# prismformore/Multi-Task-Transformer

Measured on AMD Instinct MI355X. Metric: training images/sec (512x512, 6 tasks), higher is better.
Workload: dtype f32(bf16x3)

## Files before the change

include/mtt_hip.h:

```cpp
#ifndef MTT_HIP_H
#define MTT_HIP_H

#include <stddef.h>
#include <stdint.h>

#ifdef __cplusplus
extern "C" {
#endif

#define MTT_ABI_VERSION 17

enum { MTT_F32 = 0, MTT_BF16 = 1, MTT_SPLIT = 2 };
enum { MTT_PREC_BF16 = 0, MTT_PREC_X3 = 1 };
enum { MTT_E_BADARG = -1, MTT_E_ALIGN = -2, MTT_E_UNSUPPORTED = -3 };

enum {
  MTT_OP_K = 0,
  MTT_OP_R = 1,
  MTT_OP_CONV_K = 2,
  MTT_OP_CONV_R = 3
};
enum { MTT_ACT_NONE = 0, MTT_ACT_GELU = 1, MTT_ACT_RELU = 2, MTT_ACT_GELU_BWD = 3, MTT_ACT_RELU_BWD = 4,
       MTT_ACT_GELU_DAUX = 5 ,
       MTT_ACT_MUL_AUX = 6    };
enum { MTT_STORE_ROWS = 0, MTT_STORE_PIXSHUF2 = 1 };
enum { MTT_GEMM_AUTO = 0,
       MTT_GEMM_GENERAL = 1           ,
       MTT_GEMM_DMA256 = 3            ,
       MTT_GEMM_DMA128 = 4            ,
       MTT_GEMM_GENERAL_EPILOGUE = 11  };
enum { MTT_ATTN_AUTO = 0, MTT_ATTN_PLAIN = 1,
       MTT_ATTN_FAST_V0 = 2 ,
       MTT_ATTN_FAST_V1 = 3  };

typedef struct {
  int32_t H, W;
  int32_t C;
  int32_t Cp;
  int32_t dil;
  int32_t flip;
} mtt_conv_geom;

typedef struct {
  const void* A; const void* B; void* D;
  int32_t M, N, K;
  int32_t a_op, b_op;
  int32_t a_dtype, b_dtype, d_dtype;
  int32_t prec;
  int64_t lda, ldb, ldd;
  int32_t a_mb; int64_t a_bs;
  int32_t d_mb; int64_t d_bs;
  int32_t batch, batch_inner;
  int64_t a_zo, a_zi, b_zo, b_zi, d_zo, d_zi;
  mtt_conv_geom conv;
  float alpha;
  const float* colscale; const float* colshift; int64_t col_zo, col_zi;
  int32_t act;
  const void* aux_in; void* aux_out; int32_t aux_dtype; int64_t ldaux; int64_t aux_zo, aux_zi;
  const float* rowscale; int32_t n_prompt;
  const float* resid; int64_t ldr; int32_t r_mb; int64_t r_bs; int64_t r_zo, r_zi;
  int32_t n_store;
  int32_t store_mode;
  int32_t ps_H, ps_W, ps_Co;
  int32_t variant;
  const void* A_lo; const void* B_lo; void* D_lo;
  float* colsum_out; float* colsum_ws;
  const float* a_scale; const float* a_shift; int32_t a_act; void* a_aux16; int64_t ld_a16;
} mtt_gemm_desc;
size_t mtt_gemm_colsum_ws_floats(const mtt_gemm_desc* d);

int mtt_abi_version(void);
size_t mtt_desc_size(int which);
int mtt_gemm(const mtt_gemm_desc* d, void* stream);
int mtt_gemm_variant(const mtt_gemm_desc* d);

typedef struct {
  const void* qkv; void* out; float* rawlog; float* lse;
  int32_t B, N, nH, T;
  int32_t dtype, prec;
  float scale;
  int32_t variant;
  const void* qkv_lo; void* out_lo;
} mtt_attn_desc;
int mtt_attn_fwd(const mtt_attn_desc* d, void* stream);
int mtt_attn_bwd(const mtt_attn_desc* d, const void* dout, const float* drawlog, void* dqkv, float* stat, void* stream);

typedef struct {
  const void* S; void* P; const void* dP; void* dS; const float* extra;
  int64_t rows, cols, ld; int32_t s_dtype, p_dtype; float scale;
  int64_t rows_per_mat; int32_t extra_rows; int64_t extra_ld;
} mtt_softmax_desc;
int mtt_softmax_fwd(const mtt_softmax_desc* d, void* stream);
int mtt_softmax_bwd(const mtt_softmax_desc* d, void* stream);

typedef struct {
  const float* x; void* y; const float* gamma; const float* beta; float* mean; float* rstd;
  const void* dy; float* dx; float* dgamma; float* dbeta;
  int64_t rows; int32_t C; int64_t ldx, ldy; int32_t y_dtype; float eps;
  const float* dx_in;
  float* ws;
  void* y_lo;
  float* y32; int64_t ldy32;
} mtt_ln_desc;
size_t mtt_layernorm_bwd_ws_floats(int64_t rows, int32_t C);
int mtt_layernorm_fwd(const mtt_ln_desc* d, void* stream);
int mtt_layernorm_bwd(const mtt_ln_desc* d, void* stream);

int mtt_patchify16(const float* img, void* cols, int B, int H, int W, int out_dtype, void* stream);

typedef struct {
  const void* q; const void* xn; float* rawchan;
  int32_t B, T, N, C, h, w, nh, nw; int32_t dtype; int64_t ldq;
  float* ws;
  const void* xn_lo;
} mtt_chanlogit_desc;
size_t mtt_chan_logits_ws_floats(const mtt_chanlogit_desc* d);
int mtt_chan_logits(const mtt_chanlogit_desc* d, void* stream);
int mtt_chan_logits_bwd(const mtt_chanlogit_desc* d, const float* drawchan, void* dq, int dq_dtype, float* dxn, void* stream);

typedef struct {
  const float* x; int64_t x_ld, x_bs; const float* rawlog; const float* rawchan; void* out;
  int32_t B, T, N, C, h, w, nh, nw; int32_t out_dtype;
  int32_t hg;
  void* out_lo;
} mtt_modulate_desc;
int mtt_modulate(const mtt_modulate_desc* d, void* stream);
size_t mtt_modulate_bwd_ws_floats(const mtt_modulate_desc* d);
int mtt_modulate_bwd(const mtt_modulate_desc* d, const void* dout, float* dx, float* drawlog, float* drawchan, float* ws, void* stream);

typedef struct {
  const void* fea; void* out; const float* wmix;
  int32_t T, B; int64_t rows_per_b, ld; int32_t C; int32_t fea_dtype; int32_t accumulate;
  int32_t out_dtype;
} mtt_ctr_desc;
int mtt_ctr_mix(const mtt_ctr_desc* d, void* stream);
size_t mtt_ctr_dw_ws_floats(const mtt_ctr_desc* d);
int mtt_ctr_dw(const mtt_ctr_desc* d, const float* dout, float* dwmix, float* ws, void* stream);

typedef struct {
  const float* rawlog; const float* w0; const float* b0; const float* w2; const float* b2; float* wmix;
  int32_t B, T, nH; int64_t N;
} mtt_ctrw_desc;
int mtt_ctr_weights(const mtt_ctrw_desc* d, void* stream);
int mtt_ctr_weights_bwd(const mtt_ctrw_desc* d, const float* dwmix, float* drawlog, float* dw0, float* db0, float* dw2, float* db2, void* stream);

typedef struct {
  const float* pred; const void* target; const float* weight; float* out; float* sum; float* ws;
  int64_t N; int32_t C; int32_t kind; int32_t wmode; float gamma, alpha, beta;
} mtt_detloss_desc;
size_t mtt_detloss_ws_floats(const mtt_detloss_desc* d);
int mtt_detloss_fwd(const mtt_detloss_desc* d, void* stream);
int mtt_detloss_bwd(const mtt_detloss_desc* d, const float* gscale, const float* gelem, float scale, float* dpred, void* stream);

typedef struct {
  const void* in; void* out; int32_t B, C, Hin, Win, Hout, Wout; int64_t ld_in, ld_out;
  int32_t in_dtype, out_dtype; int32_t out_nchw; int32_t accumulate;
} mtt_resize_desc;
int mtt_bilinear_fwd(const mtt_resize_desc* d, void* stream);
int mtt_bilinear_bwd(const mtt_resize_desc* d, void* stream);

typedef struct {
  const void* x; void* y; const void* dy; void* dx;
  float* mean_out; float* m2_out; const float* mean; const float* rstd; const float* gamma; const float* beta;
  float* dsum; float* dsumxh;
  int64_t rows; int32_t C; int64_t ld; int32_t dtype; int32_t act;
// ... 249 lines not shown
```

multi-task-transformer_amd/_lib.py:

```python
import ctypes as C
import os

import torch

_HERE = os.path.dirname(os.path.abspath(__file__))
LIB_PATH = os.path.join(_HERE, "libmtt_hip.so")

ABI_VERSION = 17
F32, BF16, SPLIT = 0, 1, 2
PREC_BF16, PREC_X3 = 0, 1
OP_K, OP_R, OP_CONV_K, OP_CONV_R = 0, 1, 2, 3
ACT_NONE, ACT_GELU, ACT_RELU, ACT_GELU_BWD, ACT_RELU_BWD, ACT_GELU_DAUX, ACT_MUL_AUX = 0, 1, 2, 3, 4, 5, 6
STORE_ROWS, STORE_PIXSHUF2 = 0, 1
GEMM_AUTO, GEMM_GENERAL, GEMM_DMA256, GEMM_DMA128, GEMM_GENERAL_EPILOGUE = 0, 1, 3, 4, 11
ATTN_AUTO, ATTN_PLAIN = 0, 1

i32, i64, f32, ptr = C.c_int32, C.c_int64, C.c_float, C.c_void_p


class ConvGeom(C.Structure):
    _fields_ = [("H", i32), ("W", i32), ("C", i32), ("Cp", i32), ("dil", i32), ("flip", i32)]


class GemmDesc(C.Structure):
    _fields_ = [
        ("A", ptr), ("B", ptr), ("D", ptr),
        ("M", i32), ("N", i32), ("K", i32),
        ("a_op", i32), ("b_op", i32),
        ("a_dtype", i32), ("b_dtype", i32), ("d_dtype", i32),
        ("prec", i32),
        ("lda", i64), ("ldb", i64), ("ldd", i64),
        ("a_mb", i32), ("a_bs", i64),
        ("d_mb", i32), ("d_bs", i64),
        ("batch", i32), ("batch_inner", i32),
        ("a_zo", i64), ("a_zi", i64), ("b_zo", i64), ("b_zi", i64), ("d_zo", i64), ("d_zi", i64),
        ("conv", ConvGeom),
        ("alpha", f32),
        ("colscale", ptr), ("colshift", ptr), ("col_zo", i64), ("col_zi", i64),
        ("act", i32),
        ("aux_in", ptr), ("aux_out", ptr), ("aux_dtype", i32), ("ldaux", i64), ("aux_zo", i64), ("aux_zi", i64),
        ("rowscale", ptr), ("n_prompt", i32),
        ("resid", ptr), ("ldr", i64), ("r_mb", i32), ("r_bs", i64), ("r_zo", i64), ("r_zi", i64),
        ("n_store", i32), ("store_mode", i32),
        ("ps_H", i32), ("ps_W", i32), ("ps_Co", i32),
        ("variant", i32),
        ("A_lo", ptr), ("B_lo", ptr), ("D_lo", ptr),
        ("colsum_out", ptr), ("colsum_ws", ptr),
        ("a_scale", ptr), ("a_shift", ptr), ("a_act", i32), ("a_aux16", ptr), ("ld_a16", i64),
    ]


class AttnDesc(C.Structure):
    _fields_ = [("qkv", ptr), ("out", ptr), ("rawlog", ptr), ("lse", ptr),
                ("B", i32), ("N", i32), ("nH", i32), ("T", i32), ("dtype", i32), ("prec", i32), ("scale", f32),
                ("variant", i32), ("qkv_lo", ptr), ("out_lo", ptr)]


class SoftmaxDesc(C.Structure):
    _fields_ = [("S", ptr), ("P", ptr), ("dP", ptr), ("dS", ptr), ("extra", ptr),
                ("rows", i64), ("cols", i64), ("ld", i64), ("s_dtype", i32), ("p_dtype", i32), ("scale", f32),
                ("rows_per_mat", i64), ("extra_rows", i32), ("extra_ld", i64)]


class LnDesc(C.Structure):
    _fields_ = [("x", ptr), ("y", ptr), ("gamma", ptr), ("beta", ptr), ("mean", ptr), ("rstd", ptr),
                ("dy", ptr), ("dx", ptr), ("dgamma", ptr), ("dbeta", ptr),
                ("rows", i64), ("C", i32), ("ldx", i64), ("ldy", i64), ("y_dtype", i32), ("eps", f32), ("dx_in", ptr), ("ws", ptr),
                ("y_lo", ptr), ("y32", ptr), ("ldy32", i64)]


class ChanLogitDesc(C.Structure):
    _fields_ = [("q", ptr), ("xn", ptr), ("rawchan", ptr),
                ("B", i32), ("T", i32), ("N", i32), ("C", i32), ("h", i32), ("w", i32), ("nh", i32), ("nw", i32),
                ("dtype", i32), ("ldq", i64), ("ws", ptr), ("xn_lo", ptr)]


class ModulateDesc(C.Structure):
    _fields_ = [("x", ptr), ("x_ld", i64), ("x_bs", i64), ("rawlog", ptr), ("rawchan", ptr), ("out", ptr),
                ("B", i32), ("T", i32), ("N", i32), ("C", i32), ("h", i32), ("w", i32), ("nh", i32), ("nw", i32),
                ("out_dtype", i32), ("hg", i32), ("out_lo", ptr)]


class CtrDesc(C.Structure):
    _fields_ = [("fea", ptr), ("out", ptr), ("wmix", ptr), ("T", i32), ("B", i32), ("rows_per_b", i64), ("ld", i64),
                ("C", i32), ("fea_dtype", i32), ("accumulate", i32), ("out_dtype", i32)]


class ResizeDesc(C.Structure):
    _fields_ = [("in_", ptr), ("out", ptr), ("B", i32), ("C", i32), ("Hin", i32), ("Win", i32), ("Hout", i32), ("Wout", i32),
                ("ld_in", i64), ("ld_out", i64), ("in_dtype", i32), ("out_dtype", i32), ("out_nchw", i32), ("accumulate", i32)]


class BnDesc(C.Structure):
    _fields_ = [("x", ptr), ("y", ptr), ("dy", ptr), ("dx", ptr),
                ("mean_out", ptr), ("m2_out", ptr), ("mean", ptr), ("rstd", ptr), ("gamma", ptr), ("beta", ptr),
                ("dsum", ptr), ("dsumxh", ptr),
                ("rows", i64), ("C", i32), ("ld", i64), ("dtype", i32), ("act", i32),
                ("Z", i32), ("x_zs", i64), ("p_zs", i64), ("g_dtype", i32)]


class DwconvDesc(C.Structure):
    _fields_ = [("x", ptr), ("w", ptr), ("y", ptr), ("scale", ptr), ("shift", ptr),
                ("Z", i32), ("B", i32), ("H", i32), ("W", i32), ("ld", i64), ("dtype", i32)]


class PoolDesc(C.Structure):
    _fields_ = [("x", ptr), ("y", ptr), ("B", i32), ("H", i32), ("W", i32), ("k", i32), ("ld", i64), ("dtype", i32)]


class LnMtDesc(C.Structure):
    _fields_ = [("x", ptr), ("y", ptr), ("gamma", ptr), ("beta", ptr), ("rows", i64), ("T", i32), ("D", i32),
                ("ldx", i64), ("ldy", i64), ("y_dtype", i32), ("eps", f32)]


class AttnMsgDesc(C.Structure):
    _fields_ = [("cur", ptr), ("prev", ptr), ("out", ptr), ("w", ptr), ("bias", ptr),
                ("B", i32), ("heads", i32), ("T", i32), ("qh", i32), ("qw", i32), ("K", i32), ("ldk", i64), ("ldkp", i64)]


class ConvtDesc(C.Structure):
    _fields_ = [("yall", ptr), ("out", ptr), ("bias", ptr), ("B", i32), ("H", i32), ("W", i32), ("Cop", i32),
                ("dtype", i32), ("out_dtype", i32)]


class UpconvDesc(C.Structure):
    _fields_ = [("z", ptr), ("y", ptr), ("bias", ptr), ("colscale", ptr),
                ("Z", i32), ("B", i32), ("h", i32), ("w", i32), ("C", i32), ("Cp", i32),
                ("z_dtype", i32), ("y_dtype", i32), ("act", i32)]


class AdamDesc(C.Structure):
    _fields_ = [("grads", ptr), ("params", ptr), ("exp_avg", ptr), ("exp_avg_sq", ptr), ("numel", ptr),
                ("chunk_tensor", ptr), ("chunk_off", ptr), ("n_chunks", i32),
                ("max_norm", f32), ("step_size", f32), ("beta1", f32), ("beta2", f32), ("eps", f32), ("weight_decay", f32),
                ("inv_sqrt_bc2", f32), ("hyper", ptr), ("ws", ptr)]


class LossDesc(C.Structure):
# ... 327 lines not shown
```

multi-task-transformer_amd/autograd_path.py:

```python
import math

import torch
import torch.distributed as dist
import torch.nn as nn
from torch.autograd import Function

from . import bn as bn_mod
from . import _lib, ops
from ._lib import ACT_GELU, ACT_GELU_BWD, ACT_GELU_DAUX, ACT_MUL_AUX, ACT_NONE, F32, OP_CONV_R, OP_K, OP_R, dtype_code

pitch = ops.pitch
SPLITK_MIN_ROWS = 4096
WGRAD_MAX_SLICES, WGRAD_TARGET_WGS = 192, 512


def _gemm(A, B, D, M, N, K, prec, **kw):
    args = dict(A=A, B=B, D=D, M=M, N=N, K=K, a_op=OP_K, b_op=OP_K, a_dtype=dtype_code(A), b_dtype=dtype_code(B),
                d_dtype=dtype_code(D), prec=prec.code, batch=1, batch_inner=1, alpha=1.0)
    args.update(kw)
    ops.call("gemm", **args)
    return D


def _colsum(x2d, cols):
# ... 59 lines not shown
def _wgrad_batched(dy, x, N, Kp, M, prec, Z, lda, ldb, a_zo, b_zo, a0=0, b0=0):
    A = dy.reshape(-1)[a0:] if a0 else dy
    B = x.reshape(-1)[b0:] if b0 else x
    p256 = (-(-N // 256)) * (-(-Kp // 256))
    if (prec.name == "bf16" and FAST_BWD and dy.dtype == torch.bfloat16 and x.dtype == torch.bfloat16 and M >= SPLITK_MIN_ROWS
            and min(N, Kp) >= FAST_MIN_DIM and 100 * N * Kp >= 45 * p256 * 65536 and lda % 8 == 0 and ldb % 8 == 0):
        S = _tn_splits(Z * p256, M)
        c = (M // S) // 64 * 64
        if c >= 512:
            nz = M // c
            rem = M - nz * c
            slabs = torch.empty(Z, nz + (1 if rem else 0), N, Kp, dtype=torch.float32, device=dy.device)
            SS = slabs.shape[1]
            _gemm(A, B, slabs, N, Kp, c, prec, a_op=OP_R, b_op=OP_R, lda=lda, ldb=ldb, ldd=Kp, batch=Z * nz, batch_inner=nz,
                  a_zo=a_zo, a_zi=c * lda, b_zo=b_zo, b_zi=c * ldb, d_zo=SS * N * Kp, d_zi=N * Kp)
            if rem:
                _gemm(dy.reshape(-1)[a0 + nz * c * lda:], x.reshape(-1)[b0 + nz * c * ldb:], slabs[:, nz], N, Kp, rem, prec, a_op=OP_R,
                      b_op=OP_R, lda=lda, ldb=ldb, ldd=Kp, batch=Z, a_zo=a_zo, b_zo=b_zo, d_zo=SS * N * Kp)
            return slabs.sum(1)
    tiles = Z * (-(-N // 128)) * (-(-Kp // 128))
    S = _n_splits(tiles, M // SPLIT_ROW_UNIT)
    if S == 1:
        dW = torch.empty(Z, N, Kp, dtype=torch.float32, device=dy.device)
        _gemm(A, B, dW, N, Kp, M, prec, a_op=OP_R, b_op=OP_R, lda=lda, ldb=ldb, ldd=Kp, batch=Z, a_zo=a_zo, b_zo=b_zo, d_zo=N * Kp)
        return dW
    c = (M // S) // 8 * 8
    rem = M - c * S
    slabs = torch.empty(Z, S + (1 if rem else 0), N, Kp, dtype=torch.float32, device=dy.device)
    SS = slabs.shape[1]
    _gemm(A, B, slabs, N, Kp, c, prec, a_op=OP_R, b_op=OP_R, lda=lda, ldb=ldb, ldd=Kp, batch=Z * S, batch_inner=S,
          a_zo=a_zo, a_zi=c * lda, b_zo=b_zo, b_zi=c * ldb, d_zo=SS * N * Kp, d_zi=N * Kp)
    if rem:
        _gemm(dy.reshape(-1)[a0 + c * S * lda:], x.reshape(-1)[b0 + c * S * ldb:], slabs[:, S], N, Kp, rem, prec, a_op=OP_R, b_op=OP_R,
              lda=lda, ldb=ldb, ldd=Kp, batch=Z, a_zo=a_zo, b_zo=b_zo, d_zo=SS * N * Kp)
    return slabs.sum(1)


def _pad_last(t, width):
    out = torch.zeros(t.shape[:-1] + (width,), dtype=t.dtype, device=t.device)
    out[..., :t.shape[-1]] = t
    return out


N_CUS = 256


def _tn_splits(tiles, rows, max_splits=32):
    best, cost = 2, None
    for S in range(2, max_splits + 1):
        t = -(-tiles * S // N_CUS) / S * rows * 131072 / 4.7e12 + S * tiles * 65536 * 8 / 4e12
        if cost is None or t < cost:
            best, cost = S, t
    return best


def _wgrad_tn(dy, x, N, Kp, prec):
    rows = dy.shape[0]
    lda, ldb = dy.stride(0), x.stride(0)
    tiles = -(-N // 256) * -(-Kp // 256)
    if tiles < 192 and rows >= 4096:
        S = _tn_splits(tiles, rows)
        c = (rows // S) // 64 * 64
        if c >= 512:
            nz = rows // c
            rem = rows - nz * c
            slabs = torch.empty(nz + (1 if rem else 0), N, Kp, dtype=torch.float32, device=dy.device)
            _gemm(dy, x, slabs, N, Kp, c, prec, a_op=OP_R, b_op=OP_R, lda=lda, ldb=ldb, ldd=Kp, batch=nz, a_zo=c * lda, b_zo=c * ldb, d_zo=N * Kp)
            if rem:
                _gemm(dy[nz * c:], x[nz * c:], slabs[nz], N, Kp, rem, prec, a_op=OP_R, b_op=OP_R, lda=lda, ldb=ldb, ldd=Kp)
            return slabs.sum(0)
    dW = torch.empty(N, Kp, dtype=torch.float32, device=dy.device)
    return _gemm(dy, x, dW, N, Kp, rows, prec, a_op=OP_R, b_op=OP_R, lda=lda, ldb=ldb, ldd=Kp)


def _enc_wgrad(dy, x, N, Kp, prec, bias=True):
    db = _colsum(dy, N) if bias else None
    if (prec.name == "bf16" and FAST_BWD and N >= FAST_MIN_DIM and Kp >= FAST_MIN_DIM and dy.shape[0] >= FAST_MIN_ROWS
            and N % 8 == 0 and dy.stride(0) % 8 == 0):
        if dy.dtype == torch.bfloat16 and x.dtype == torch.bfloat16:
            return _wgrad_tn(dy, x, N, Kp, prec), db
    return _wgrad(dy, x, N, Kp, prec), db


def _enc_dgrad(dy, weight, wpack2d, M, N_in, K_out, prec, out_dtype, tag, colsum=False, **epi):
    if colsum:
        if prec.name == "bf16" and (dy.dtype != torch.bfloat16 or wpack2d.dtype != torch.bfloat16):
            dx = _enc_dgrad(dy, weight, wpack2d, M, N_in, K_out, prec, out_dtype, tag, **epi)
            return dx, _colsum(dx, N_in)
        cs = torch.empty(N_in, dtype=torch.float32, device=dy.device)
        epi = dict(epi, colsum_out=cs, colsum_ws=ops.ws_for("gemm_colsum", dy.device, M=M, N=N_in))
        return _enc_dgrad(dy, weight, wpack2d, M, N_in, K_out, prec, out_dtype, tag, **epi), cs
    if prec.name == "bf16" and FAST_BWD and dy.dtype == torch.bfloat16 and K_out % 64 == 0 and N_in >= FAST_MIN_DIM:
        wT = ops.pack_linear_T(weight, torch.bfloat16, tag)
        dx = torch.empty(M, N_in, dtype=out_dtype, device=dy.device)
        return _gemm(dy, wT, dx, M, N_in, K_out, prec, lda=dy.stride(0), ldb=wT.stride(0), ldd=N_in, n_store=N_in, **epi)
    return _dgrad(dy, wpack2d, M, N_in, K_out, prec, out_dtype, **epi)


FAST_BWD = True
GELU_DAUX = True
FAST_MIN_DIM, FAST_MIN_ROWS = 256, 1024


def _dgrad(dy, wpack2d, M, N_in, K_out, prec, out_dtype, **epi):
    dx = torch.empty(M, N_in, dtype=out_dtype, device=dy.device)
    return _gemm(dy, wpack2d, dx, M, N_in, K_out, prec, b_op=OP_R, lda=dy.stride(0), ldb=wpack2d.stride(0), ldd=N_in,
                 n_store=N_in, **epi)


def layernorm(x, gamma, beta, eps, prec, out_dtype, keep):
    if keep:
        return LayerNormFn.apply(x, gamma, beta, eps, prec, out_dtype)
    return ops.layernorm(x, gamma, beta, eps, prec, out_dtype=out_dtype)[0]


class LayerNormFn(Function):
    @staticmethod
    def forward(ctx, x, gamma, beta, eps, prec, out_dtype):
        y, mean, rstd = ops.layernorm(x, gamma, beta, eps, prec, save_stats=True, out_dtype=out_dtype)
        ctx.save_for_backward(x, gamma, mean, rstd)
        ctx.eps = eps
        return y

    @staticmethod
    def backward(ctx, dy):
        x, gamma, mean, rstd = ctx.saved_tensors
        dy = dy.contiguous()
        dx, dg, db = torch.zeros_like(x), torch.empty_like(gamma), torch.empty_like(gamma)
        ops.call("layernorm_bwd", x=x, dy=dy, gamma=gamma, mean=mean, rstd=rstd, dx=dx, dgamma=dg, dbeta=db,
                 rows=x.shape[0], C=x.shape[1], ldx=x.stride(0), ldy=dy.stride(0), y_dtype=dtype_code(dy), eps=ctx.eps,
                 ws=ops.ln_bwd_ws(x.shape[0], x.shape[1], x.device))
        return dx, dg, db, None, None, None


def attention_bwd(qkv, dao, drawlog, B, N, nH, T, prec):
    C, Np, Z = nH * 64, pitch(N), B * nH
    dev, adt = qkv.device, prec.adt
    scale = 64 ** -0.5
    S = torch.empty(Z, N, Np, dtype=adt, device=dev)
    zS = dict(batch=Z, batch_inner=nH, d_zo=nH * N * Np, d_zi=N * Np)
    zq = dict(a_zo=N * 3 * C, a_zi=64)
    _gemm(qkv, qkv[:, C:], S, N, N, 64, prec, lda=3 * C, ldb=3 * C, ldd=Np, b_zo=N * 3 * C, b_zi=64, n_store=Np, **zq, **zS)
    ops.call("softmax_fwd", S=S, P=S, rows=Z * N, cols=N, ld=Np, s_dtype=dtype_code(S), p_dtype=dtype_code(S), scale=scale)
    dP = torch.empty(Z, N, Np, dtype=adt, device=dev)
    _gemm(dao, qkv[:, 2 * C:], dP, N, N, 64, prec, lda=C, ldb=3 * C, ldd=Np, a_zo=N * C, a_zi=64, b_zo=N * 3 * C, b_zi=64,
          n_store=Np, **zS)
    ops.call("softmax_bwd", P=S, dP=dP, dS=dP, extra=drawlog, rows=Z * N, cols=N, ld=Np, s_dtype=dtype_code(S),
             p_dtype=dtype_code(S), scale=scale, rows_per_mat=N, extra_rows=T if drawlog is not None else 0, extra_ld=N)
    dqkv = torch.empty(B * N, 3 * C, dtype=adt, device=dev)
    zP = dict(batch=Z, batch_inner=nH, a_zo=nH * N * Np, a_zi=N * Np, d_zo=N * 3 * C, d_zi=64)
    _gemm(S, dao, dqkv[:, 2 * C:], N, 64, N, prec, a_op=OP_R, b_op=OP_R, lda=Np, ldb=C, ldd=3 * C, b_zo=N * C, b_zi=64, **zP)
    _gemm(dP, qkv[:, C:], dqkv, N, 64, N, prec, b_op=OP_R, lda=Np, ldb=3 * C, ldd=3 * C, b_zo=N * 3 * C, b_zi=64, **zP)
    _gemm(dP, qkv, dqkv[:, C:], N, 64, N, prec, a_op=OP_R, b_op=OP_R, lda=Np, ldb=3 * C, ldd=3 * C, b_zo=N * 3 * C, b_zi=64, **zP)
    return dqkv


HEAD_DGRAD_DMA = True
FLASH_BWD = True


def attention_bwd_flash(qkv, ao, lse, dao, drawlog, B, N, nH, T, prec):
    dqkv = torch.empty_like(qkv)
    dsum = torch.empty(B, nH, 2, (N + 3) // 4 * 4, dtype=torch.float32, device=qkv.device)
    ops.call("attn_bwd", qkv=qkv, out=ao, rawlog=None, lse=lse, B=B, N=N, nH=nH, T=T, dtype=dtype_code(qkv), prec=prec.code,
             scale=64 ** -0.5, xargs=[dao, drawlog, dqkv, dsum])
    return dqkv


def _ln_bwd_join(dres, x, dy, gamma, mean, rstd, eps):
    dg, db = torch.empty_like(gamma), torch.empty_like(gamma)
    out = torch.empty_like(dres)
    ops.call("layernorm_bwd", x=x, dy=dy, gamma=gamma, mean=mean, rstd=rstd, dx=out, dx_in=dres, dgamma=dg, dbeta=db,
             rows=x.shape[0], C=x.shape[1], ldx=x.stride(0), ldy=dy.stride(0), y_dtype=dtype_code(dy), eps=eps,
             ws=ops.ln_bwd_ws(x.shape[0], x.shape[1], x.device))
    return out, dg, db


def attn_half(XT, g1, b1, eps, Wqkv, bqkv, Wproj, bproj, Wtt, btt, Wtt1, btt1, rowscale, geo, prec, tag, *, keep, gp=None):
    B, N, nH, T, h, w, nwin = geo[:7]
    side = geo[7] if len(geo) > 7 else True
    pe, pa, ps = gp or (prec, prec, prec)
    assert not keep or pe.name == pa.name == ps.name == prec.name, "per-group precisions are inference-only"
    C, hw = nH * 64, h * w
    chan = Wtt is not None
    split = prec.split
    odt = "split" if split else prec.adt
    xn, mean, rstd = ops.layernorm(XT, g1, b1, eps, prec, save_stats=keep, out_dtype=odt)
    wq = ops.pack_linear([Wqkv], pe, tag + ('qkv',), split=split)
    wp = ops.pack_linear([Wproj], pe, tag + ('proj',), split=split)
    qkv = ops.linear(xn, wq, 3 * C, pe, bias=bqkv[None], out_dtype=odt)[0]
    flash = keep and (split or (FLASH_BWD and prec.name == "bf16" and qkv.dtype == torch.bfloat16))
    if not split and pa.adt != qkv.dtype:
        q16 = ops.cast2d(qkv, qkv.shape[0], 3 * C, 3 * C, pa.adt, ldd=3 * C)
        ao16, rawlog, lse = ops.attention(q16, B, N, nH, T, pa)
        ao = ops.cast2d(ao16, ao16.shape[0], C, C, prec.adt, ldd=C)
    else:
        ao, rawlog, lse = ops.attention(qkv, B, N, nH, T, pa, want_lse=flash)
    XT2 = torch.empty_like(XT)
    rows = dict(d_rows=(N, N * C, C), M=B * N) if keep or rowscale is not None else {}
    ops.linear(ao, wp, C, pe, bias=bproj[None], out=XT2, resid=XT, rowscale=rowscale, n_prompt=T, **rows)
    cq = wt = wt1 = xp32 = rawchan = None
    if chan:
        wt = ops.pack_linear([Wtt], ps, tag + ('tt',))
        wt1 = ops.pack_linear([Wtt1], ps, tag + ('tt1',))
        if split:
            xp32 = ops.prompt_rows32(xn, B, N, T, C)
            cq = ops.linear(xp32, wt, hw, ps, bias=btt[None], M=B * T)[0]
        else:
            cq = ops.linear(xn, wt, hw, ps, bias=btt[None], a_rows=(T, N * C, C), M=B * T)[0]
        if side:
            xnc = xn if split or ps.adt == xn.dtype else ops.cast2d(xn, xn.shape[0], C, C, ps.adt, ldd=C)
            rawchan = ops.chan_logits(cq, xnc, B, T, N, C, (h, w), (nwin, nwin))
        pr = XT2.view(B, N, C)[:, :T]
        ops.linear(cq, wt1, C, ps, bias=btt1[None], out=pr, d_rows=(T, N * C, C), resid=pr, rowscale=rowscale, n_prompt=T, M=B * T)
    saved = (XT, g1, mean, rstd, ops._hi(xn), ops._hi(qkv), ops._hi(ao), ops._hi(wq), ops._hi(wp), rowscale, lse, cq, wt, wt1, xp32) if keep else None
    return (XT2, rawlog, rawchan), saved


def mlp_half(XT2, g2, b2n, eps, W1, b1, W2, b2, rowscale, geo, prec, tag, *, keep, pe=None):
    B, N, T = geo
    pe = pe or prec
    assert not keep or pe.name == prec.name
    C, Hd = W1.shape[1], W1.shape[0]
    split = prec.split and ((C % 64 == 0 and Hd % 64 == 0) if MLP_SPLIT_RULE64 else (ops.split_gemm_ok(C) and ops.split_gemm_ok(Hd)))
    odt = "split" if split else prec.adt
    xn2, mean, rstd = ops.layernorm(XT2, g2, b2n, eps, prec, save_stats=keep, out_dtype=odt)
    w1 = ops.pack_linear([W1], pe, tag + ('fc1',), split=split)
    w2 = ops.pack_linear([W2], pe, tag + ('fc2',), split=split)
    z = torch.empty(B * N, Hd, dtype=prec.bwd.adt, device=XT2.device) if keep else None
    daux = keep and GELU_DAUX and z.dtype == torch.bfloat16
    hmid = ops.linear(xn2, w1, Hd, pe, bias=b1[None], act=ACT_GELU_DAUX if daux else ACT_GELU, aux_out=z, out_dtype=odt)[0]
    XT3 = torch.empty_like(XT2)
    rows = dict(d_rows=(N, N * C, C), M=B * N) if keep or rowscale is not None else {}
    ops.linear(hmid, w2, C, pe, bias=b2[None], out=XT3, resid=XT2, rowscale=rowscale, n_prompt=T, **rows)
    saved = (XT2, g2, mean, rstd, ops._hi(xn2), z, ops._hi(hmid), ops._hi(w1), ops._hi(w2), rowscale) if keep else None
    return XT3, saved


class AttnHalfFn(Function):

    @staticmethod
    def forward(ctx, XT, g1, b1, eps, Wqkv, bqkv, Wproj, bproj, Wtt, btt, Wtt1, btt1, rowscale, geo, prec, tag):
        (XT2, rawlog, rawchan), saved = attn_half(XT, g1, b1, eps, Wqkv, bqkv, Wproj, bproj, Wtt, btt, Wtt1, btt1, rowscale, geo, prec, tag, keep=True)
        ctx.save_for_backward(*saved)
        ctx.geo, ctx.prec, ctx.eps, ctx.chan = geo, prec, eps, Wtt is not None
        ctx.params = (Wqkv, Wproj, Wtt, Wtt1)
        ctx.set_materialize_grads(False)
        z = torch.zeros(0, device=XT.device)
        return XT2, (rawlog if rawlog is not None else z), (rawchan if rawchan is not None else z)

    @staticmethod
    def backward(ctx, dXT2, drawlog, drawchan):
        XT, g1, mean, rstd, xn, qkv, ao, wq, wp, rowscale, lse, cq, wt, wt1, xp32 = ctx.saved_tensors
        Wqkv_, Wproj_, Wtt_, Wtt1_ = ctx.params
        B, N, nH, T, h, w, nwin = ctx.geo[:7]
        prec, C, M, hw = ctx.prec.bwd, nH * 64, B * N, h * w
        xn_c = xn
        if dXT2 is None:
            dXT2 = torch.zeros_like(XT)
        dXT2 = dXT2.contiguous()
        g, dbproj = _scaled_colsum(dXT2, rowscale, N, T, prec)
        dWproj, _ = _enc_wgrad(g, ao, C, C, prec, bias=False)
        dao = _enc_dgrad(g, Wproj_, wp[0], M, C, C, prec, prec.adt, 'proj')
        dl = drawlog.contiguous() if (T > 0 and drawlog is not None and drawlog.numel()) else None
        if lse is not None:
            dqkv = attention_bwd_flash(qkv, ao, lse, dao, dl, B, N, nH, T, prec)
        else:
            dqkv = attention_bwd(qkv, dao, dl, B, N, nH, T, prec)
        dWqkv, dbqkv = _enc_wgrad(dqkv, xn, 3 * C, C, prec)
        dxn = _enc_dgrad(dqkv, Wqkv_, wq[0], M, C, 3 * C, prec, torch.float32, 'qkv')
        dWtt = dbtt = dWtt1 = dbtt1 = None
        if ctx.chan:
            hwp = cq.shape[-1]
            gp = dXT2.view(B, N, C)[:, :T].reshape(B * T, C)
            if rowscale is not None:
                gp = gp * rowscale[:, 0].repeat_interleave(T)[:, None]
            dWtt1 = _wgrad(gp, cq, C, hwp, prec)[:, :hw]
            dbtt1 = _colsum(gp, C)
            fast_tt = prec.name == "bf16" and FAST_BWD and hwp == hw and hw >= FAST_MIN_DIM and C >= FAST_MIN_DIM and C % 64 == 0
            if fast_tt:
                gp16 = ops.cast_rows(gp, torch.bfloat16)
                dcq = _enc_dgrad(gp16, Wtt1_, wt1[0], B * T, hwp, C, prec, torch.float32, 'tt1')
            else:
                dcq = _dgrad(gp, wt1[0], B * T, hwp, C, prec, torch.float32)
            if drawchan is not None and drawchan.numel():
                dq2 = torch.zeros(B * T, hwp, dtype=torch.float32, device=xn.device)
                cqb = cq if cq.dtype == xn_c.dtype else ops.cast_rows(cq, xn_c.dtype)
                ops.call("chan_logits_bwd", q=cqb, xn=xn_c, rawchan=None, B=B, T=T, N=N, C=C, h=h, w=w, nh=nwin, nw=nwin,
                         dtype=dtype_code(xn_c), ldq=hwp, xargs=[drawchan.contiguous(), dq2, F32, dxn])
                dcq = dcq + dq2
            xnp = xp32 if xp32 is not None else xn_c.view(B, N, C)[:, :T].reshape(B * T, C)
            dWtt = _wgrad(dcq, xnp, hw, C, prec)[:, :C]
            dbtt = _colsum(dcq, hw)
            dp = dxn.view(B, N, C)[:, :T]
            if fast_tt:
                dcq16 = ops.cast_rows(dcq, torch.bfloat16)
                wT = ops.pack_linear_T(Wtt_, torch.bfloat16, 'tt')
                _gemm(dcq16, wT, dp, B * T, C, hw, prec, lda=hwp, ldb=hw, ldd=C, d_mb=T, d_bs=N * C,
                      resid=dp, r_mb=T, r_bs=N * C, ldr=C, n_store=C)
            else:
                _gemm(dcq, wt[0], dp, B * T, C, hw, prec, b_op=OP_R, lda=hwp, ldb=wt.shape[-1], ldd=C, d_mb=T, d_bs=N * C,
                      resid=dp, r_mb=T, r_bs=N * C, ldr=C, n_store=C)
        dXT, dg1, db1 = _ln_bwd_join(dXT2, XT, dxn, g1, mean, rstd, ctx.eps)
        return (dXT, dg1, db1, None, dWqkv, dbqkv, dWproj, dbproj, dWtt, dbtt, dWtt1, dbtt1, None, None, None, None)


class MlpHalfFn(Function):

    @staticmethod
    def forward(ctx, XT2, g2, b2n, eps, W1, b1, W2, b2, rowscale, geo, prec, tag):
        XT3, saved = mlp_half(XT2, g2, b2n, eps, W1, b1, W2, b2, rowscale, geo, prec, tag, keep=True)
        ctx.save_for_backward(*saved)
        ctx.geo, ctx.prec, ctx.eps, ctx.daux = geo, prec, eps, GELU_DAUX and saved[5].dtype == torch.bfloat16
        ctx.params = (W1, W2)
        return XT3

    @staticmethod
    def backward(ctx, dXT3):
        XT2, g2, mean, rstd, xn2, z, hmid, w1, w2, rowscale = ctx.saved_tensors
        B, N, T = ctx.geo
        prec, M = ctx.prec.bwd, B * N
        C, Hd = xn2.shape[1], z.shape[1]
        dXT3 = dXT3.contiguous()
        g, db2 = _scaled_colsum(dXT3, rowscale, N, T, prec)
        W1_, W2_ = ctx.params
        dW2, _ = _enc_wgrad(g, hmid, C, Hd, prec, bias=False)
        dz, db1 = _enc_dgrad(g, W2_, w2[0], M, Hd, C, prec, prec.adt, 'fc2', colsum=True, act=ACT_MUL_AUX if ctx.daux else ACT_GELU_BWD, aux_in=z,
                             aux_dtype=dtype_code(z), ldaux=Hd)
        dW1, _ = _enc_wgrad(dz, xn2, Hd, C, prec, bias=False)
        dxn2 = _enc_dgrad(dz, W1_, w1[0], M, C, Hd, prec, prec.adt, 'fc1')
        dXT2, dg2, dbn2 = _ln_bwd_join(dXT3, XT2, dxn2, g2, mean, rstd, ctx.eps)
        return dXT2, dg2, dbn2, None, dW1, db1, dW2, db2, None, None, None, None


def block_attn(keep, gp, *args):
    return AttnHalfFn.apply(*args) if keep else attn_half(*args, keep=False, gp=gp)[0]


def block_mlp(keep, pe, *args):
    return MlpHalfFn.apply(*args) if keep else mlp_half(*args, keep=False, pe=pe)[0]


def patch_embed(img, Wpe, bpe, pos, first, geo, prec, tag, pe=None):
    B, N, T, hw = geo
    C = Wpe.shape[0]
    XT = torch.empty(B * N, C, dtype=torch.float32, device=img.device)
    XT.view(B, N, C)[:, :T] = first
    cols = ops.patchify(img.float(), prec)
    wpe = ops.pack_linear([Wpe], pe or prec, tag)
    ops.linear(cols, wpe, C, pe or prec, bias=bpe[None], out=XT.view(B, N, C)[:, T:], d_rows=(hw, N * C, C),
               resid=pos[0, 1:], r_rows=(hw, 0, C), M=B * hw)
    return XT, cols


class PatchEmbedFn(Function):

    @staticmethod
    def forward(ctx, img, Wpe, bpe, pos, prompts, geo, prec):
        XT, cols = patch_embed(img, Wpe, bpe, pos, prompts, geo, prec, 'pe')
        ctx.save_for_backward(cols)
        ctx.geo, ctx.prec, ctx.wshape = geo, prec, Wpe.shape
        return XT

    @staticmethod
    def backward(ctx, dXT):
        (cols,) = ctx.saved_tensors
        B, N, T, hw = ctx.geo
        C = ctx.wshape[0]
        d3 = dXT.contiguous().view(B, N, C)
        dpatch = d3[:, T:].reshape(B * hw, C)
        dW = _wgrad(dpatch, cols, C, 768, ctx.prec.bwd).view(ctx.wshape)
        db = _colsum(dpatch, C)
        dpos = torch.zeros(1, hw + 1, C, dtype=torch.float32, device=dXT.device)
        dpos[0, 1:] = d3[:, T:].sum(0)
        return None, dW, db, dpos, d3[:, :T].sum(0), None, None


class ModulateFn(Function):

    @staticmethod
    def forward(ctx, xsrc, rawlog, rawchan, geo, prec, split=False):
        B, N, T, C, h, w, nwin = geo[:7]
        hg = geo[7] if len(geo) > 7 else 0
        mod = ops.modulate(xsrc.view(B, N, C)[:, T:], C, N * C, rawlog, rawchan, B, T, N, C, (h, w), (nwin, nwin), prec, hg=hg, split=split)
        ctx.save_for_backward(xsrc, rawlog, rawchan)
        ctx.geo = geo
        if split:
            ctx.mark_non_differentiable(mod.lo)
            ctx.set_materialize_grads(False)
            return mod.hi, mod.lo
        return mod

    @staticmethod
    def backward(ctx, dmod, *_):
        xsrc, rawlog, rawchan = ctx.saved_tensors
        B, N, T, C, h, w, nwin = ctx.geo[:7]
        hg = ctx.geo[7] if len(ctx.geo) > 7 else 0
        dmod = dmod.contiguous()
        dx = torch.empty_like(xsrc)
        dx.view(B, N, C)[:, :T].zero_()
        dl, dc = torch.zeros_like(rawlog), torch.empty_like(rawchan)
        ops.call("modulate_bwd", x=xsrc.view(B, N, C)[:, T:], x_ld=C, x_bs=N * C, rawlog=rawlog, rawchan=rawchan, out=None,
                 B=B, T=T, N=N, C=C, h=h, w=w, nh=nwin, nw=nwin, out_dtype=dtype_code(dmod), hg=hg,
                 xargs=[dmod, dx.view(B, N, C)[:, T:], dl, dc, ops.ws_for("modulate_bwd", dmod.device, B=B, T=T, C=C, h=h, w=w, nh=nwin, nw=nwin)])
        return dx, dl, dc, None, None, None


MLP_SPLIT_RULE64 = False
AUTO_SPLIT = True
AUTO_SPLIT_MIN_ROWS = 2048


class BLinearFn(Function):
# ... 640 lines not shown
```

multi-task-transformer_amd/csrc/attn_bwd.hip:

```cpp
#include "mtt_device.h"
#include <type_traits>

#ifndef MTT_ABWD_TILES
#define MTT_ABWD_TILES 1
#endif
#ifndef MTT_ABWD_STATDMA
#define MTT_ABWD_STATDMA 1
#endif
#ifndef MTT_ABWD_DQSTAT
#define MTT_ABWD_DQSTAT 1
#endif

namespace {

constexpr int HD = 64;
constexpr int KTILE = 64 * HD * 2;
constexpr float LOG2E = 1.4426950408889634f;

struct BwdP {
  const bf16_t* qkv; const bf16_t* dout; const float* stat; const float* drawlog; bf16_t* dqkv;
  int B, N, nH, T, Np; float scale;
  const bf16_t* out; const float* lse; float* stat_w;
};

MTT_DEV float dot8_bf16(const u32x4& a, const u32x4& g) {
  float s = 0.f;
#pragma unroll
  for (int j = 0; j < 4; ++j) s += lo_of(a[j]) * lo_of(g[j]) + hi_of(a[j]) * hi_of(g[j]);
  return s;
}

__global__ __launch_bounds__(256) void attn_stat_kernel(const bf16_t* out, const bf16_t* dout, const float* lse, float* stat, int B, int N,
                                                        int nH, int Np) {
  const int C8 = nH * 8;
  const int64_t total = (int64_t)B * N * C8;
  const int64_t t = (int64_t)blockIdx.x * 256 + threadIdx.x;
  float s = 0.f;
  if (t < total) {
    const u32x4 a = *(const u32x4*)(out + t * 8), g = *(const u32x4*)(dout + t * 8);
    s = dot8_bf16(a, g);
  }
  s += __shfl_xor(s, 1, 64); s += __shfl_xor(s, 2, 64); s += __shfl_xor(s, 4, 64);
  if (t < total && (threadIdx.x & 7) == 0) {
    const int64_t tok = t / C8;
    const int h = (int)(t % C8) >> 3;
    const int b = (int)(tok / N), n = (int)(tok % N);
    float* row = stat + ((int64_t)b * nH + h) * 2 * Np;
    row[n] = s;
    row[Np + n] = lse[((int64_t)b * nH + h) * N + n] * LOG2E;
    if (n == N - 1)
      for (int k = N; k < Np; ++k) { row[k] = 0.f; row[Np + k] = 0.f; }
  }
}

MTT_DEV u32x4 perm_frag(const unsigned char* tile, int row, int ks, int lg) {
  const u32x2 lo = *(const u32x2*)(tile + lds_off(row, 4 * ks + (lg >> 1)) + (lg & 1) * 8);
  const u32x2 hi = *(const u32x2*)(tile + lds_off(row, 4 * ks + 2 + (lg >> 1)) + (lg & 1) * 8);
  return (u32x4){lo[0], lo[1], hi[0], hi[1]};
}

template <bool TR>
MTT_DEV void store_units(unsigned char* rowmajor, unsigned char* transposed, const u32x4 (&sh)[4], int kq, int rb) {
#pragma unroll
  for (int i = 0; i < 4; ++i) *(u32x4*)(rowmajor + lds_off(kq * 4 + i, rb)) = sh[i];
  if (TR) {
    u32x2 piece[8];
    transpose4x8(sh, piece);
#pragma unroll
    for (int j = 0; j < 8; ++j) *(u32x2*)(transposed + lds_off(rb * 8 + j, kq >> 1) + (kq & 1) * 8) = piece[j];
  }
}

__device__ __attribute__((aligned(32))) const unsigned g_bwd_zero_page[8] = {0u, 0u, 0u, 0u, 0u, 0u, 0u, 0u};
MTT_DEV int bwd_swz(int row) { return (((row >> 1) & 3) << 1) | ((row >> 3) & 1); }
MTT_DEV void bwd_glds16(const bf16_t* src, unsigned char* lds_wave_base) {
  __builtin_amdgcn_global_load_lds((const __attribute__((address_space(1))) void*)src,
                                   (__attribute__((address_space(3))) void*)lds_wave_base, 16, 0, 0);
}
MTT_DEV void bwd_glds4(const float* src, unsigned char* lds_wave_base) {
  __builtin_amdgcn_global_load_lds((const __attribute__((address_space(1))) void*)src,
                                   (__attribute__((address_space(3))) void*)lds_wave_base, 4, 0, 0);
}
using BwdDyn = std::integral_constant<int, -1>;
using BwdNo = std::integral_constant<int, 0>;
using BwdYes = std::integral_constant<int, 1>;
template <int OFF>
MTT_DEV u32x2 bwd_ds_read_tr16(unsigned addr) {
  u32x2 r;
  asm volatile("ds_read_b64_tr_b16 %0, %1 offset:%2" : "=v"(r) : "v"(addr), "n"(OFF) : "memory");
  return r;
}
template <int OFF>
MTT_DEV f32x4 bwd_ds_read_f4(unsigned addr) {
  f32x4 r;
  asm volatile("ds_read_b128 %0, %1 offset:%2" : "=v"(r) : "v"(addr), "n"(OFF) : "memory");
  return r;
}
#define BWD_TRW(x) "+v"(x)
#define BWD_WAIT_TR8(a, b)                                                                                                              \
  asm volatile("s_waitcnt lgkmcnt(0)" : BWD_TRW(a[0]), BWD_TRW(a[1]), BWD_TRW(a[2]), BWD_TRW(a[3]), BWD_TRW(b[0]), BWD_TRW(b[1]), BWD_TRW(b[2]), BWD_TRW(b[3]) :: "memory")
#define BWD_WAIT_TR16(a, b, c, d)                                                                                                       \
  asm volatile("s_waitcnt lgkmcnt(0)" : BWD_TRW(a[0]), BWD_TRW(a[1]), BWD_TRW(a[2]), BWD_TRW(a[3]), BWD_TRW(b[0]), BWD_TRW(b[1]), BWD_TRW(b[2]), BWD_TRW(b[3]), \
               BWD_TRW(c[0]), BWD_TRW(c[1]), BWD_TRW(c[2]), BWD_TRW(c[3]), BWD_TRW(d[0]), BWD_TRW(d[1]), BWD_TRW(d[2]), BWD_TRW(d[3]) :: "memory")
#define BWD_WAIT_TR16_F4(a, b, c, d, e, f)                                                                                              \
  asm volatile("s_waitcnt lgkmcnt(0)" : BWD_TRW(a[0]), BWD_TRW(a[1]), BWD_TRW(a[2]), BWD_TRW(a[3]), BWD_TRW(b[0]), BWD_TRW(b[1]), BWD_TRW(b[2]), BWD_TRW(b[3]), \
               BWD_TRW(c[0]), BWD_TRW(c[1]), BWD_TRW(c[2]), BWD_TRW(c[3]), BWD_TRW(d[0]), BWD_TRW(d[1]), BWD_TRW(d[2]), BWD_TRW(d[3]),                       \
               BWD_TRW(e[0]), BWD_TRW(e[1]), BWD_TRW(f[0]), BWD_TRW(f[1]) :: "memory")

template <int VER>
__global__ __launch_bounds__(256, 2) void attn_bwd_dq_kernel(const BwdP p) {
  extern __shared__ __attribute__((aligned(16))) unsigned char smem[];
  constexpr int STAGE = (VER == 2 ? 2 : 3) * KTILE;
  const int nqb = (p.N + 127) / 128;
  const int wi = xcd_remap(blockIdx.x, gridDim.x);
  const int qb = wi % nqb, bh_ = wi / nqb;
  const int h = bh_ % p.nH, b = bh_ / p.nH;
  const int N = p.N, C = p.nH * HD;
  const int tid = threadIdx.x, lane = tid & 63, wave = tid >> 6;
  const int li = lane & 15, lg = lane >> 4;
  const int64_t tok0 = (int64_t)b * N;
  const int64_t bh = (int64_t)b * p.nH + h;
  const int q0 = qb * 128 + wave * 32;
  const bool active = q0 < N;

  u32x4 qf[2][2], gf[2][2], dummy;
  float lse2[2], Dq[2];
#pragma unroll
  for (int sub = 0; sub < 2; ++sub) {
    const int qrow = q0 + sub * 16 + li;
    const bool ok = qrow < N;
#pragma unroll
    for (int kh = 0; kh < 2; ++kh) {
      Raw8<false> r;
      load8_raw<false>(p.qkv, (tok0 + qrow) * 3 * C + h * HD + kh * 32 + lg * 8, ok, r);
      cvt8<false, false>(ok, r, qf[sub][kh], dummy);
      load8_raw<false>(p.dout, (tok0 + qrow) * C + h * HD + kh * 32 + lg * 8, ok, r);
      cvt8<false, false>(ok, r, gf[sub][kh], dummy);
    }
    if constexpr (VER == 2 && MTT_ABWD_DQSTAT) {
      float c[2];
#pragma unroll
      for (int kh = 0; kh < 2; ++kh) {
        Raw8<false> r;
        u32x4 of;
        load8_raw<false>(p.out, (tok0 + qrow) * C + h * HD + kh * 32 + lg * 8, ok, r);
        cvt8<false, false>(ok, r, of, dummy);
        c[kh] = dot8_bf16(of, gf[sub][kh]);
        c[kh] += __shfl_xor(c[kh], 16, 64);
        c[kh] += __shfl_xor(c[kh], 32, 64);
      }
      Dq[sub] = c[0] + c[1];
      lse2[sub] = ok ? p.lse[bh * N + qrow] * LOG2E : 0.f;
      if (ok && lg == 0) {
        p.stat_w[bh * 2 * p.Np + qrow] = Dq[sub];
        p.stat_w[bh * 2 * p.Np + p.Np + qrow] = lse2[sub];
      }
    } else {
      Dq[sub] = ok ? p.stat[bh * 2 * p.Np + qrow] : 0.f;
      lse2[sub] = ok ? p.stat[bh * 2 * p.Np + p.Np + qrow] : 0.f;
    }
  }
  if constexpr (VER == 2 && MTT_ABWD_DQSTAT) {
    if (qb == nqb - 1 && tid < p.Np - N) {
      p.stat_w[bh * 2 * p.Np + N + tid] = 0.f;
      p.stat_w[bh * 2 * p.Np + p.Np + N + tid] = 0.f;
    }
  }

  const bool isK = tid < 128;
  const int kq = tid & 15, rb = (tid >> 4) & 7;
  Raw8<false> raw[4];
  unsigned okm = 0;
  auto stage_load = [&](int kv0) {
    if (VER >= 1 && kv0 + 64 <= N) {
      okm = 0xfu;
#pragma unroll
      for (int i = 0; i < 4; ++i)
        raw[i].r0 = *(const u32x4*)(p.qkv + ((tok0 + kv0 + kq * 4 + i) * 3 * C + (isK ? C : 2 * C) + h * HD + rb * 8));
      return;
    }
    okm = 0;
#pragma unroll
    for (int i = 0; i < 4; ++i) {
      const int key = kv0 + kq * 4 + i;
      const bool ok = key < N;
      okm |= (ok ? 1u : 0u) << i;
      load8_raw<false>(p.qkv, (tok0 + key) * 3 * C + (isK ? C : 2 * C) + h * HD + rb * 8, ok, raw[i]);
    }
  };
  auto stage_store = [&](unsigned char* st) {
    u32x4 sh[4];
    if (VER >= 1 && okm == 0xfu) {
#pragma unroll
      for (int i = 0; i < 4; ++i) sh[i] = raw[i].r0;
    } else {
#pragma unroll
      for (int i = 0; i < 4; ++i) cvt8<false, false>((okm >> i) & 1u, raw[i], sh[i], dummy);
    }
    if (isK) store_units<true>(st, st + KTILE, sh, kq, rb);
    else store_units<false>(st + 2 * KTILE, nullptr, sh, kq, rb);
  };

  int dma_off[4], dma_row[2];
  uint64_t zpage = 0;
// ... 259 lines not shown
    for (int i = 0; i < 4; ++i) {
      const int row = q0 + kq * 4 + i;
      const bool ok = row < N;
      okm |= (ok ? 1u : 0u) << i;
      if (isQ) load8_raw<false>(p.qkv, (tok0 + row) * 3 * C + h * HD + rb * 8, ok, raw[i]);
      else load8_raw<false>(p.dout, (tok0 + row) * C + h * HD + rb * 8, ok, raw[i]);
    }
  };
  auto stage_store = [&](unsigned char* st) {
    u32x4 sh[4];
    if (VER >= 1 && okm == 0xfu) {
#pragma unroll
      for (int i = 0; i < 4; ++i) sh[i] = raw[i].r0;
    } else {
#pragma unroll
      for (int i = 0; i < 4; ++i) cvt8<false, false>((okm >> i) & 1u, raw[i], sh[i], dummy);
    }
    unsigned char* base = isQ ? st : st + 2 * KTILE;
    store_units<true>(base, base + KTILE, sh, kq, rb);
  };

  int dma_off[4], dma_row[2];
  uint64_t zpage = 0;
  unsigned taddr[4];
  const unsigned char* faddr[2];
  if (VER == 2) {
    zpage = (uint64_t)(uintptr_t)g_bwd_zero_page;
    asm volatile("" : "+s"(zpage));
#pragma unroll
    for (int i = 0; i < 2; ++i) {
      const int r = wave * 16 + i * 8 + (lane >> 3), pc = lane & 7;
      dma_row[i] = r;
      dma_off[i] = r * 3 * C + ((pc ^ bwd_swz(r)) & 7) * 8;
      dma_off[2 + i] = r * C + ((pc ^ bwd_swz(r)) & 7) * 8;
    }
    const int trow = 4 * lg + (li >> 2);
#pragma unroll
    for (int dt = 0; dt < 4; ++dt)
      taddr[dt] = (unsigned)(uintptr_t)smem + (unsigned)(trow * 128 + (((2 * dt + ((li & 3) >> 1)) ^ bwd_swz(trow)) & 7) * 16 + (li & 1) * 8);
#pragma unroll
    for (int kh = 0; kh < 2; ++kh) faddr[kh] = smem + li * 128 + (((kh * 4 + lg) ^ bwd_swz(li)) & 7) * 16;
  }
  const float* Drow = p.stat + bh * 2 * p.Np;
  const float* Lrow = Drow + p.Np;
  constexpr int STAT_LDS = 2 * STAGE, STAT_STAGE = 2 * 64 * 4;
  const unsigned saddr = (unsigned)(uintptr_t)smem + (unsigned)(lg * 16);
  auto dma_issue = [&](unsigned char* st, unsigned char* sst, int q0) {
    if (MTT_ABWD_STATDMA && __builtin_amdgcn_readfirstlane(wave) < 2) {
      const float* src = (wave ? Lrow : Drow) + q0 + lane;
      if (q0 + 64 > p.Np) src = q0 + lane < p.Np ? src : (const float*)(uintptr_t)zpage;
      bwd_glds4(src, sst + wave * 256);
    }
    const bf16_t* baseQ = p.qkv + ((tok0 + q0) * 3 * C + h * HD);
    const bf16_t* baseG = p.dout + ((tok0 + q0) * C + h * HD);
    unsigned char* dQ = st + wave * 2048;
    unsigned char* dG = st + KTILE + wave * 2048;
    if (q0 + 64 <= N) {
#pragma unroll
      for (int i = 0; i < 2; ++i) bwd_glds16(baseQ + dma_off[i], dQ + i * 1024);
#pragma unroll
      for (int i = 0; i < 2; ++i) bwd_glds16(baseG + dma_off[2 + i], dG + i * 1024);
    } else {
#pragma unroll
      for (int i = 0; i < 2; ++i) {
        const bool ok = q0 + dma_row[i] < N;
        bwd_glds16((const bf16_t*)(uintptr_t)(ok ? (uint64_t)(uintptr_t)(baseQ + dma_off[i]) : zpage), dQ + i * 1024);
      }
#pragma unroll
      for (int i = 0; i < 2; ++i) {
        const bool ok = q0 + dma_row[i] < N;
        bwd_glds16((const bf16_t*)(uintptr_t)(ok ? (uint64_t)(uintptr_t)(baseG + dma_off[2 + i]) : zpage), dG + i * 1024);
      }
    }
  };

  f32x4 dk[2][4], dv[2][4];
#pragma unroll
  for (int kt = 0; kt < 2; ++kt)
#pragma unroll
    for (int t = 0; t < 4; ++t) { dk[kt][t] = (f32x4){0.f, 0.f, 0.f, 0.f}; dv[kt][t] = (f32x4){0.f, 0.f, 0.f, 0.f}; }
  const float sc2 = p.scale * LOG2E, inv_scale = 1.0f / p.scale;

  const int nq = (N + 63) / 64;
  if (VER == 2) {
    dma_issue(smem, smem + STAT_LDS, 0);
    asm volatile("s_waitcnt vmcnt(0)" ::: "memory");
  } else {
    stage_load(0);
    stage_store(smem);
  }
  __syncthreads();

  auto tile = [&](auto stage_tag, auto ragged_tag, auto first_tag, int j) {
    constexpr int ST = decltype(stage_tag)::value;
    constexpr int RG = decltype(ragged_tag)::value, FT = decltype(first_tag)::value;
    const bool more = RG != 1 && j + 1 < nq;
    if (more) {
      if (VER == 2) dma_issue(smem + (1 - ST) * STAGE, smem + STAT_LDS + (1 - ST) * STAT_STAGE, (j + 1) * 64);
      else stage_load((j + 1) * 64);
    }
    const unsigned char* Qh = smem + (ST < 0 ? (j & 1) : ST) * STAGE;
    const unsigned char* Qt = Qh + KTILE;
    const unsigned char* Gh = Qh + 2 * KTILE;
    const unsigned char* Gt = Qh + 3 * KTILE;
    const int q0 = j * 64;
    if (active) {
      const bool full = RG < 0 ? q0 + 64 <= N : RG == 0;
      const bool add_raw = FT != 0 && p.drawlog != nullptr && (FT > 0 || j == 0) && p.T > 0;
#pragma unroll
      for (int ks = 0; ks < 2; ++ks) {
        if (RG != 0 && q0 + 32 * ks >= N) continue;
        f32x4 s[2][2], dp[2][2];
        f32x4 D4[2], L4[2];
        u32x2 qtl[4], qth[4], gtl[4], gth[4];
        if constexpr (VER == 2) {
          constexpr bool LATE = RG == 1;
          u32x4 qa[2][2], ga[2][2];
          auto read_stat = [&]() {
#pragma unroll
            for (int q2 = 0; q2 < 2; ++q2) {
              D4[q2] = bwd_ds_read_f4<STAT_LDS + ST * STAT_STAGE>(saddr + (ks ? 128 : 0) + q2 * 64);
              L4[q2] = bwd_ds_read_f4<STAT_LDS + ST * STAT_STAGE + 256>(saddr + (ks ? 128 : 0) + q2 * 64);
            }
          };
          auto read_tr = [&]() {
            if (ks == 0) {
#pragma unroll
              for (int dt = 0; dt < 4; ++dt) {
                qtl[dt] = bwd_ds_read_tr16<ST * STAGE>(taddr[dt]); qth[dt] = bwd_ds_read_tr16<ST * STAGE + 16 * 128>(taddr[dt]);
                gtl[dt] = bwd_ds_read_tr16<ST * STAGE + KTILE>(taddr[dt]); gth[dt] = bwd_ds_read_tr16<ST * STAGE + KTILE + 16 * 128>(taddr[dt]);
              }
            } else {
#pragma unroll
              for (int dt = 0; dt < 4; ++dt) {
                qtl[dt] = bwd_ds_read_tr16<ST * STAGE + 32 * 128>(taddr[dt]); qth[dt] = bwd_ds_read_tr16<ST * STAGE + 48 * 128>(taddr[dt]);
                gtl[dt] = bwd_ds_read_tr16<ST * STAGE + KTILE + 32 * 128>(taddr[dt]); gth[dt] = bwd_ds_read_tr16<ST * STAGE + KTILE + 48 * 128>(taddr[dt]);
              }
            }
          };
          auto wait_reads = [&]() {
            if constexpr (MTT_ABWD_STATDMA) BWD_WAIT_TR16_F4(qtl, qth, gtl, gth, D4, L4);
            else BWD_WAIT_TR16(qtl, qth, gtl, gth);
          };
          if constexpr (MTT_ABWD_STATDMA && !LATE) read_stat();
#pragma unroll
          for (int q2 = 0; q2 < 2; ++q2) {
            if constexpr (!MTT_ABWD_STATDMA) {
              const int qr = q0 + (2 * ks + q2) * 16 + lg * 4;
              D4[q2] = qr < p.Np ? *(const f32x4*)(Drow + qr) : (f32x4){0.f, 0.f, 0.f, 0.f};
              L4[q2] = qr < p.Np ? *(const f32x4*)(Lrow + qr) : (f32x4){0.f, 0.f, 0.f, 0.f};
            }
#pragma unroll
            for (int kh = 0; kh < 2; ++kh) {
              qa[q2][kh] = *(const u32x4*)(faddr[kh] + ST * STAGE + q2 * 2048 + (ks ? 4096 : 0));
              ga[q2][kh] = *(const u32x4*)(faddr[kh] + ST * STAGE + KTILE + q2 * 2048 + (ks ? 4096 : 0));
            }
          }
          if constexpr (!LATE) { read_tr(); wait_reads(); }
          __builtin_amdgcn_s_setprio(1);
#pragma unroll
          for (int q2 = 0; q2 < 2; ++q2) {
#pragma unroll
            for (int kt = 0; kt < 2; ++kt) { s[q2][kt] = (f32x4){0.f, 0.f, 0.f, 0.f}; dp[q2][kt] = (f32x4){0.f, 0.f, 0.f, 0.f}; }
#pragma unroll
            for (int kh = 0; kh < 2; ++kh)
#pragma unroll
              for (int kt = 0; kt < 2; ++kt) {
                s[q2][kt] = mfma16(qa[q2][kh], kf[kt][kh], s[q2][kt]);
                dp[q2][kt] = mfma16(ga[q2][kh], vf[kt][kh], dp[q2][kt]);
              }
          }
          __builtin_amdgcn_s_setprio(0);
          if constexpr (LATE) {
            if constexpr (MTT_ABWD_STATDMA) read_stat();
            read_tr();
            wait_reads();
          }
        } else {
        if (VER >= 1) __builtin_amdgcn_s_setprio(1);
#pragma unroll
        for (int q2 = 0; q2 < 2; ++q2) {
          const int qs = 2 * ks + q2;
          const int qr = q0 + qs * 16 + lg * 4;
          D4[q2] = qr < p.Np ? *(const f32x4*)(Drow + qr) : (f32x4){0.f, 0.f, 0.f, 0.f};
          L4[q2] = qr < p.Np ? *(const f32x4*)(Lrow + qr) : (f32x4){0.f, 0.f, 0.f, 0.f};
#pragma unroll
          for (int kt = 0; kt < 2; ++kt) { s[q2][kt] = (f32x4){0.f, 0.f, 0.f, 0.f}; dp[q2][kt] = (f32x4){0.f, 0.f, 0.f, 0.f}; }
#pragma unroll
          for (int kh = 0; kh < 2; ++kh) {
            const u32x4 qa = *(const u32x4*)(Qh + lds_off(qs * 16 + li, kh * 4 + lg));
            const u32x4 ga = *(const u32x4*)(Gh + lds_off(qs * 16 + li, kh * 4 + lg));
#pragma unroll
            for (int kt = 0; kt < 2; ++kt) {
              s[q2][kt] = mfma16(qa, kf[kt][kh], s[q2][kt]);
              dp[q2][kt] = mfma16(ga, vf[kt][kh], dp[q2][kt]);
            }
          }
        }
        if (VER >= 1) __builtin_amdgcn_s_setprio(0);
        }
        u32x4 pb[2], dsb[2];
#pragma unroll
        for (int kt = 0; kt < 2; ++kt) {
          float pv[2][4], ds[2][4];
#pragma unroll
          for (int q2 = 0; q2 < 2; ++q2) {
            const float lr[4] = {L4[q2][0], L4[q2][1], L4[q2][2], L4[q2][3]};
            const float dr[4] = {D4[q2][0], D4[q2][1], D4[q2][2], D4[q2][3]};
#pragma unroll
            for (int r = 0; r < 4; ++r) {
              pv[q2][r] = __builtin_amdgcn_exp2f(fmaf(s[q2][kt][r], sc2, -lr[r]));
              if (!full && q0 + (2 * ks + q2) * 16 + lg * 4 + r >= N) pv[q2][r] = 0.f;
              ds[q2][r] = pv[q2][r] * (dp[q2][kt][r] - dr[r]);
            }
          }
          if (add_raw && ks == 0) {
            const int key = key0 + kt * 16 + li;
#pragma unroll
            for (int r = 0; r < 4; ++r) {
              const int q = lg * 4 + r;
              if (q < p.T && key < N) ds[0][r] += p.drawlog[(bh * p.T + q) * N + key] * inv_scale;
            }
          }
          pb[kt] = (u32x4){pack2(pv[0][0], pv[0][1]), pack2(pv[0][2], pv[0][3]), pack2(pv[1][0], pv[1][1]), pack2(pv[1][2], pv[1][3])};
          dsb[kt] = (u32x4){pack2(ds[0][0], ds[0][1]), pack2(ds[0][2], ds[0][3]), pack2(ds[1][0], ds[1][1]), pack2(ds[1][2], ds[1][3])};
        }
        if (VER >= 1) __builtin_amdgcn_s_setprio(1);
#pragma unroll
        for (int dt = 0; dt < 4; ++dt) {
          u32x4 ga, qa;
          if constexpr (VER == 2) {
            ga = (u32x4){gtl[dt][0], gtl[dt][1], gth[dt][0], gth[dt][1]};
            qa = (u32x4){qtl[dt][0], qtl[dt][1], qth[dt][0], qth[dt][1]};
          } else {
            ga = perm_frag(Gt, dt * 16 + li, ks, lg);
            qa = perm_frag(Qt, dt * 16 + li, ks, lg);
          }
#pragma unroll
          for (int kt = 0; kt < 2; ++kt) {
            dv[kt][dt] = mfma16(ga, pb[kt], dv[kt][dt]);
            dk[kt][dt] = mfma16(qa, dsb[kt], dk[kt][dt]);
          }
        }
        if (VER >= 1) __builtin_amdgcn_s_setprio(0);
      }
    }
    if (more) {
      if (VER == 2) asm volatile("s_waitcnt vmcnt(0)" ::: "memory");
      else stage_store(smem + (ST < 0 ? ((j + 1) & 1) : (1 - ST)) * STAGE);
    }
    __syncthreads();
  };
  if (VER == 2 && MTT_ABWD_TILES) {
    const int nfull = N / 64;
    if (nfull >= 1) tile(BwdNo{}, BwdNo{}, BwdYes{}, 0);
    else tile(BwdNo{}, BwdYes{}, BwdYes{}, 0);
    for (int j = 1; j < nfull; j += 2) {
      tile(BwdYes{}, BwdNo{}, BwdNo{}, j);
      if (j + 1 < nfull) tile(BwdNo{}, BwdNo{}, BwdNo{}, j + 1);
    }
    if (nfull >= 1 && nfull < nq) {
      if (nfull & 1) tile(BwdYes{}, BwdYes{}, BwdNo{}, nfull);
      else tile(BwdNo{}, BwdYes{}, BwdNo{}, nfull);
    }
  } else if (VER >= 1) {
    for (int j = 0; j < nq; j += 2) {
      tile(BwdNo{}, BwdDyn{}, BwdDyn{}, j);
      if (j + 1 < nq) tile(BwdYes{}, BwdDyn{}, BwdDyn{}, j + 1);
    }
  } else {
    for (int j = 0; j < nq; ++j) tile(BwdDyn{}, BwdDyn{}, BwdDyn{}, j);
  }
  int tid_e = tid;
  asm volatile("" : "+v"(tid_e));
  const int li_e = tid_e & 15, lg_e = (tid_e >> 4) & 3, key0_e = kb * 128 + (tid_e >> 6) * 32;
#pragma unroll
  for (int kt = 0; kt < 2; ++kt) {
    const int krow = key0_e + kt * 16 + li_e;
    if (krow >= N) continue;
#pragma unroll
    for (int dt = 0; dt < 4; ++dt) {
      bf16_t* dst = p.dqkv + (tok0 + krow) * 3 * C + C + h * HD + dt * 16 + lg_e * 4;
      *(u32x2*)dst = (u32x2){pack2(dk[kt][dt][0] * p.scale, dk[kt][dt][1] * p.scale), pack2(dk[kt][dt][2] * p.scale, dk[kt][dt][3] * p.scale)};
      *(u32x2*)(dst + C) = (u32x2){pack2(dv[kt][dt][0], dv[kt][dt][1]), pack2(dv[kt][dt][2], dv[kt][dt][3])};
    }
  }
}

}

extern "C" int mtt_attn_bwd(const mtt_attn_desc* d, const void* dout, const float* drawlog, void* dqkv, float* stat, void* stream) {
  if (!d || !d->qkv || !d->out || !d->lse || !dout || !dqkv || !stat) return MTT_E_BADARG;
  if (d->B <= 0 || d->N <= 0 || d->nH <= 0 || d->T < 0 || d->T > 16) return MTT_E_BADARG;
  if (d->dtype != MTT_BF16 || d->prec != MTT_PREC_BF16) return MTT_E_UNSUPPORTED;
  if (((uintptr_t)d->qkv | (uintptr_t)dout | (uintptr_t)d->out | (uintptr_t)stat | (uintptr_t)dqkv) & 15) return MTT_E_ALIGN;
  hipStream_t s = (hipStream_t)stream;
  constexpr int smem_dq = 2 * 3 * KTILE, smem_dkv = 2 * 4 * KTILE, smem_dma = 2 * 2 * KTILE;
  constexpr int smem_dma_dkv = smem_dma + (MTT_ABWD_STATDMA ? 2 * 2 * 64 * 4 : 0);
  static std::atomic<unsigned long long> done_dq0{0}, done_dkv0{0}, done_dq1{0}, done_dkv1{0};
  const int ver = d->variant == MTT_ATTN_FAST_V0 ? 0 : d->variant == MTT_ATTN_FAST_V1 ? 1 : 2;
  if (ver == 0) {
    if (int e = mtt_ensure_dyn_lds((const void*)attn_bwd_dq_kernel<0>, smem_dq, done_dq0)) return e;
    if (int e = mtt_ensure_dyn_lds((const void*)attn_bwd_dkv_kernel<0>, smem_dkv, done_dkv0)) return e;
  } else if (ver == 1) {
    if (int e = mtt_ensure_dyn_lds((const void*)attn_bwd_dq_kernel<1>, smem_dq, done_dq1)) return e;
    if (int e = mtt_ensure_dyn_lds((const void*)attn_bwd_dkv_kernel<1>, smem_dkv, done_dkv1)) return e;
  }
  const int Np = (d->N + 3) & ~3;
  const int64_t chunks = (int64_t)d->B * d->N * d->nH * 8;
  if (ver != 2 || !MTT_ABWD_DQSTAT)
    hipLaunchKernelGGL(attn_stat_kernel, dim3((unsigned)((chunks + 255) / 256)), dim3(256), 0, s, (const bf16_t*)d->out, (const bf16_t*)dout,
                       d->lse, stat, d->B, d->N, d->nH, Np);
  BwdP p{(const bf16_t*)d->qkv, (const bf16_t*)dout, stat, d->T > 0 ? drawlog : nullptr, (bf16_t*)dqkv, d->B, d->N, d->nH, d->T, Np, d->scale,
         (const bf16_t*)d->out, d->lse, stat};
  dim3 grid((unsigned)(((d->N + 127) / 128) * d->nH * d->B));
  if (ver == 0) {
    hipLaunchKernelGGL(attn_bwd_dq_kernel<0>, grid, dim3(256), smem_dq, s, p);
    hipLaunchKernelGGL(attn_bwd_dkv_kernel<0>, grid, dim3(256), smem_dkv, s, p);
  } else if (ver == 1) {
    hipLaunchKernelGGL(attn_bwd_dq_kernel<1>, grid, dim3(256), smem_dq, s, p);
    hipLaunchKernelGGL(attn_bwd_dkv_kernel<1>, grid, dim3(256), smem_dkv, s, p);
  } else {
    hipLaunchKernelGGL(attn_bwd_dq_kernel<2>, grid, dim3(256), smem_dma, s, p);
    hipLaunchKernelGGL(attn_bwd_dkv_kernel<2>, grid, dim3(256), smem_dma_dkv, s, p);
  }
  return (int)hipGetLastError();
}
```

multi-task-transformer_amd/csrc/attn_fast.hip:

```cpp
#include "mtt_device.h"
#include <type_traits>

namespace {

constexpr int KV = 64, HD = 64;
constexpr int KTILE = KV * HD * 2;
constexpr float LOG2E = 1.4426950408889634f;

struct AttnP { mtt_attn_desc d; };

MTT_DEV u32x4 perm_frag(const unsigned char* tile, int row, int ks, int lg) {
  const u32x2 lo = *(const u32x2*)(tile + lds_off(row, 4 * ks + (lg >> 1)) + (lg & 1) * 8);
  const u32x2 hi = *(const u32x2*)(tile + lds_off(row, 4 * ks + 2 + (lg >> 1)) + (lg & 1) * 8);
  return (u32x4){lo[0], lo[1], hi[0], hi[1]};
}

__device__ __attribute__((aligned(32))) const unsigned g_attn_zero_page[8] = {0u, 0u, 0u, 0u, 0u, 0u, 0u, 0u};
MTT_DEV void attn_glds16(const bf16_t* src, unsigned char* lds_wave_base) {
  __builtin_amdgcn_global_load_lds((const __attribute__((address_space(1))) void*)src,
                                   (__attribute__((address_space(3))) void*)lds_wave_base, 16, 0, 0);
}
template <int OFF>
MTT_DEV u32x2 attn_ds_read_tr16(unsigned addr) {
  u32x2 r;
  asm volatile("ds_read_b64_tr_b16 %0, %1 offset:%2" : "=v"(r) : "v"(addr), "n"(OFF) : "memory");
  return r;
}
template <int VER>
__global__ __launch_bounds__(256, 2) void attn_fwd_fast_kernel(const AttnP p) {
  extern __shared__ __attribute__((aligned(16))) unsigned char smem[];
  constexpr int STAGE = 2 * KTILE;
  const mtt_attn_desc& d = p.d;
  const int nqb = (d.N + 127) / 128;
  const int wi = xcd_remap(blockIdx.x, gridDim.x);
  const int qb = wi % nqb, bh = wi / nqb;
  const int h = bh % d.nH, b = bh / d.nH;
  const int N = d.N, C = d.nH * HD;
  const int tid = threadIdx.x, lane = tid & 63, wave = tid >> 6;
  const int li = lane & 15, lg = lane >> 4;
  const int64_t tok0 = (int64_t)b * N;
  const bf16_t* qkv = (const bf16_t*)d.qkv;
  const int q0 = qb * 128 + wave * 32;
  const bool active = q0 < N;

  u32x4 qf[2][2], dummy;
#pragma unroll
  for (int sub = 0; sub < 2; ++sub) {
    const int qrow = q0 + sub * 16 + li;
    const bool ok = qrow < N;
#pragma unroll
    for (int kh = 0; kh < 2; ++kh) {
      Raw8<false> r;
      load8_raw<false>(qkv, (tok0 + qrow) * 3 * C + h * HD + kh * 32 + lg * 8, ok, r);
      cvt8<false, false>(ok, r, qf[sub][kh], dummy);
    }
  }

  const bool isV = tid < 128;
  Raw8<false> raw[4];
  unsigned okm = 0;
  const int kq = tid & 15, rb = (tid >> 4) & 7;
  const int kt_ = tid - 128;
  auto stage_load = [&](int kv0) {
    if (VER >= 1 && kv0 + KV <= N) {
      okm = 0xfu;
#pragma unroll
      for (int i = 0; i < 4; ++i) {
        const int idx = kt_ + 128 * i;
        const int key = isV ? kv0 + kq * 4 + i : kv0 + (idx >> 3);
        const int col = isV ? 2 * C + rb * 8 : C + (idx & 7) * 8;
        raw[i].r0 = *(const u32x4*)(qkv + ((tok0 + key) * 3 * C + col + h * HD));
      }
      return;
    }
    okm = 0;
#pragma unroll
    for (int i = 0; i < 4; ++i) {
      const int idx = kt_ + 128 * i;
      const int key = isV ? kv0 + kq * 4 + i : kv0 + (idx >> 3);
      const int col = isV ? 2 * C + rb * 8 : C + (idx & 7) * 8;
      const bool ok = key < N;
      okm |= (ok ? 1u : 0u) << i;
      load8_raw<false>(qkv, (tok0 + key) * 3 * C + col + h * HD, ok, raw[i]);
    }
  };
  auto stage_store = [&](unsigned char* st) {
    u32x4 sh[4];
    if (VER >= 1 && okm == 0xfu) {
#pragma unroll
      for (int i = 0; i < 4; ++i) sh[i] = raw[i].r0;
    } else {
#pragma unroll
      for (int i = 0; i < 4; ++i) cvt8<false, false>((okm >> i) & 1u, raw[i], sh[i], dummy);
    }
    if (isV) {
      u32x2 piece[8];
      transpose4x8(sh, piece);
#pragma unroll
      for (int j = 0; j < 8; ++j) *(u32x2*)(st + KTILE + lds_off(rb * 8 + j, kq >> 1) + (kq & 1) * 8) = piece[j];
    } else {
#pragma unroll
      for (int i = 0; i < 4; ++i) {
        const int idx = kt_ + 128 * i;
        *(u32x4*)(st + lds_off(idx >> 3, idx & 7)) = sh[i];
      }
    }
  };

  int dma_off[4];
  int dma_row[2];
  uint64_t zpage = 0;
  if (VER >= 2) {
    zpage = (uint64_t)(uintptr_t)g_attn_zero_page;
    asm volatile("" : "+s"(zpage));
#pragma unroll
    for (int i = 0; i < 2; ++i) {
      const int r = wave * 16 + i * 8 + (lane >> 3), pc = lane & 7;
      dma_row[i] = r;
      dma_off[i] = r * 3 * C + C + ((pc ^ (r >> 1)) & 7) * 8;
// ... 168 lines not shown
        }
#define ATW(x) "+v"(x)
        asm volatile("s_waitcnt lgkmcnt(8)"
                     : ATW(v0l[0]), ATW(v0l[1]), ATW(v0l[2]), ATW(v0l[3]), ATW(v0h[0]), ATW(v0h[1]), ATW(v0h[2]), ATW(v0h[3]),
                       ATW(v1l[0]), ATW(v1l[1]), ATW(v1l[2]), ATW(v1l[3]), ATW(v1h[0]), ATW(v1h[1]), ATW(v1h[2]), ATW(v1h[3]) :: "memory");
        __builtin_amdgcn_s_setprio(1);
#pragma unroll
        for (int dt = 0; dt < 4; ++dt) {
          const u32x4 vf = (u32x4){v0l[dt][0], v0l[dt][1], v0h[dt][0], v0h[dt][1]};
          o[0][dt] = mfma16(vf, pb[0][0], o[0][dt]);
          o[1][dt] = mfma16(vf, pb[1][0], o[1][dt]);
        }
        asm volatile("s_waitcnt lgkmcnt(0)" : ATW(v1l[0]), ATW(v1l[1]), ATW(v1l[2]), ATW(v1l[3]), ATW(v1h[0]), ATW(v1h[1]), ATW(v1h[2]), ATW(v1h[3]) :: "memory");
        if (half1) {
#pragma unroll
          for (int dt = 0; dt < 4; ++dt) {
            const u32x4 vf = (u32x4){v1l[dt][0], v1l[dt][1], v1h[dt][0], v1h[dt][1]};
            o[0][dt] = mfma16(vf, pb[0][1], o[0][dt]);
            o[1][dt] = mfma16(vf, pb[1][1], o[1][dt]);
          }
        }
        __builtin_amdgcn_s_setprio(0);
#undef ATW
      } else {
      if (VER >= 1) __builtin_amdgcn_s_setprio(1);
#pragma unroll
      for (int ks = 0; ks < 2; ++ks) {
        if (kv0 + 32 * ks >= N) continue;
#pragma unroll
        for (int dt = 0; dt < 4; ++dt) {
          const u32x4 vf = perm_frag(Vt, dt * 16 + li, ks, lg);
          o[0][dt] = mfma16(vf, pb[0][ks], o[0][dt]);
          o[1][dt] = mfma16(vf, pb[1][ks], o[1][dt]);
        }
      }
      if (VER >= 1) __builtin_amdgcn_s_setprio(0);
      }
    }
    if (more) {
      if (VER >= 2) asm volatile("s_waitcnt vmcnt(0)" ::: "memory");
      else stage_store(smem + (ST < 0 ? ((j + 1) & 1) : (1 - ST)) * STAGE);
    }
    __syncthreads();
  };
  if (VER >= 1) {
    for (int j = 0; j < nkv; j += 2) {
      tile(std::integral_constant<int, 0>{}, j);
      if (j + 1 < nkv) tile(std::integral_constant<int, 1>{}, j + 1);
    }
  } else {
    for (int j = 0; j < nkv; ++j) tile(std::integral_constant<int, -1>{}, j);
  }

  bf16_t* out = (bf16_t*)d.out;
#pragma unroll
  for (int sub = 0; sub < 2; ++sub) {
    float l = l_part[sub];
    if (VER >= 2) {
      l = groups_sum(l);
    } else {
      l += __shfl_xor(l, 16, 64);
      l += __shfl_xor(l, 32, 64);
    }
    const int qrow = q0 + sub * 16 + li;
    if (qrow >= N) continue;
    const float inv = 1.0f / l;
#pragma unroll
    for (int dt = 0; dt < 4; ++dt)
      *(u32x2*)(out + (tok0 + qrow) * C + h * HD + dt * 16 + lg * 4) =
          (u32x2){pack2(o[sub][dt][0] * inv, o[sub][dt][1] * inv), pack2(o[sub][dt][2] * inv, o[sub][dt][3] * inv)};
    if (d.lse && lg == 0) d.lse[((int64_t)b * d.nH + h) * N + qrow] = (m_run[sub] + log2f(l)) * 0.6931471805599453f;
  }
}


__global__ __launch_bounds__(256, 2) void attn_fwd_x3_kernel(const AttnP p) {
  extern __shared__ __attribute__((aligned(16))) unsigned char smem[];
  constexpr int STAGE = 4 * KTILE;
  const mtt_attn_desc& d = p.d;
  const int nqb = (d.N + 127) / 128;
  const int wi = xcd_remap(blockIdx.x, gridDim.x);
  const int qb = wi % nqb, bh = wi / nqb;
  const int h = bh % d.nH, b = bh / d.nH;
  const int N = d.N, C = d.nH * HD;
  const int tid = threadIdx.x, lane = tid & 63, wave = tid >> 6;
  const int li = lane & 15, lg = lane >> 4;
  const int64_t tok0 = (int64_t)b * N;
  const bf16_t* qh_ = (const bf16_t*)d.qkv;
  const bf16_t* ql_ = (const bf16_t*)d.qkv_lo;
  const int q0 = qb * 128 + wave * 32;
  const bool active = q0 < N;

  u32x4 qfh[2][2], qfl[2][2];
#pragma unroll
  for (int sub = 0; sub < 2; ++sub) {
    const int qrow = q0 + sub * 16 + li;
    const bool ok = qrow < N;
    const int64_t qi = (tok0 + (ok ? qrow : 0)) * 3 * C + h * HD + lg * 8;
#pragma unroll
    for (int kh = 0; kh < 2; ++kh) {
      const u32x4 z = (u32x4){0u, 0u, 0u, 0u};
      qfh[sub][kh] = ok ? *(const u32x4*)(qh_ + qi + kh * 32) : z;
      qfl[sub][kh] = ok ? *(const u32x4*)(ql_ + qi + kh * 32) : z;
    }
  }

  int dma_off[4], dma_row[2];
  uint64_t zpage = (uint64_t)(uintptr_t)g_attn_zero_page;
  asm volatile("" : "+s"(zpage));
#pragma unroll
  for (int i = 0; i < 2; ++i) {
    const int r = wave * 16 + i * 8 + (lane >> 3), pc = lane & 7;
    dma_row[i] = r;
    dma_off[i] = r * 3 * C + C + ((pc ^ (r >> 1)) & 7) * 8;
    dma_off[2 + i] = r * 3 * C + 2 * C + (((((pc >> 1) ^ (r >> 1)) & 3) << 1) | (pc & 1)) * 8;
  }
  auto dma_issue = [&](unsigned char* st, int kv0) {
    const int64_t boff = (tok0 + kv0) * 3 * C + h * HD;
    const bool full = kv0 + KV <= N;
#pragma unroll
    for (int pl = 0; pl < 2; ++pl) {
      const bf16_t* base = (pl ? ql_ : qh_) + boff;
#pragma unroll
      for (int kv = 0; kv < 2; ++kv) {
        unsigned char* dst = st + (kv * 2 + pl) * KTILE + wave * 2048;
#pragma unroll
        for (int i = 0; i < 2; ++i) {
          const bool ok = full || kv0 + dma_row[i] < N;
          attn_glds16((const bf16_t*)(uintptr_t)(ok ? (uint64_t)(uintptr_t)(base + dma_off[kv * 2 + i]) : zpage), dst + i * 1024);
        }
      }
    }
  };
  const int vrow = 4 * lg + (li >> 2);
  const int vf_ = (vrow >> 1) & 3;
  unsigned vaddr[4];
#pragma unroll
  for (int dt = 0; dt < 4; ++dt) vaddr[dt] = (unsigned)(uintptr_t)smem + (unsigned)(2 * KTILE + vrow * 128 + (li & 3) * 8 + ((dt ^ vf_) & 3) * 32);
  const unsigned char* kaddr[2];
#pragma unroll
  for (int kh = 0; kh < 2; ++kh) kaddr[kh] = smem + li * 128 + (((kh * 4 + lg) ^ (li >> 1)) & 7) * 16;

  f32x4 o[2][4];
#pragma unroll
  for (int sub = 0; sub < 2; ++sub)
#pragma unroll
    for (int t = 0; t < 4; ++t) o[sub][t] = (f32x4){0.f, 0.f, 0.f, 0.f};
  float m_run[2] = {-INFINITY, -INFINITY}, l_part[2] = {0.f, 0.f};
  const float sc2 = d.scale * LOG2E;
  const bool write_raw = d.rawlog != nullptr && d.T > 0 && qb == 0 && wave == 0 && li < d.T;

  const int nkv = (N + KV - 1) / KV;
  dma_issue(smem, 0);
  asm volatile("s_waitcnt vmcnt(0)" ::: "memory");
  __syncthreads();

  auto tile = [&](auto stage_tag, int j) {
    constexpr int ST = decltype(stage_tag)::value;
    const bool more = j + 1 < nkv;
    if (more) dma_issue(smem + (1 - ST) * STAGE, (j + 1) * KV);
    const int kv0 = j * KV;
    if (active) {
      f32x4 s[2][4];
      {
        u32x4 kf[4][2];
#pragma unroll
// ... 196 lines not shown
```

multi-task-transformer_amd/csrc/gemm.hip:

```cpp
#include "mtt_device.h"
#include <type_traits>

namespace {

#ifndef MTT_GROUP_M
#define MTT_GROUP_M 4
#endif
#ifndef MTT_RING
#define MTT_RING 1
#endif
constexpr int BM = 128, BN = 128, BK = 64;
constexpr int TILE_BYTES = BM * BK * 2;

struct GemmP {
  mtt_gemm_desc d;
  FastDiv divW, divH, divCp, div3;
  FastDiv divAmb, divDmb, divRmb;
  FastDiv divPsW, divPsH, divPsCo;
  int tiles_m, tiles_n;
  int group_m;
#ifdef MTT_GEMM_TRACE
  unsigned long long* trace;
#endif
};

#ifdef MTT_GEMM_TRACE
MTT_DEV unsigned long long trace_hwid() {
  unsigned a, b;
  asm volatile("s_getreg_b32 %0, hwreg(HW_REG_HW_ID)" : "=s"(a));
  asm volatile("s_getreg_b32 %0, hwreg(HW_REG_XCC_ID)" : "=s"(b));
  return (unsigned long long)a | ((unsigned long long)b << 32);
}
#define MTT_TRACE(slot) do { if (p.trace && threadIdx.x == 0) p.trace[(size_t)(blockIdx.x + gridDim.x * blockIdx.z) * 8 + (slot)] = __builtin_amdgcn_s_memtime(); } while (0)
#define MTT_TRACE_RT(slot) do { if (p.trace && threadIdx.x == 0) p.trace[(size_t)(blockIdx.x + gridDim.x * blockIdx.z) * 8 + (slot)] = __builtin_amdgcn_s_memrealtime(); } while (0)
#define MTT_TRACE_ID(tile) do { if (p.trace && threadIdx.x == 0) { p.trace[(size_t)(blockIdx.x + gridDim.x * blockIdx.z) * 8 + 6] = trace_hwid(); p.trace[(size_t)(blockIdx.x + gridDim.x * blockIdx.z) * 8 + 7] = (tile); } } while (0)
#else
#define MTT_TRACE(slot) do {} while (0)
#define MTT_TRACE_RT(slot) do {} while (0)
#define MTT_TRACE_ID(tile) do {} while (0)
#endif

MTT_DEV int64_t row_off(uint32_t m, int mb, int64_t bs, int64_t ld, FastDiv f) {
  if (mb <= 0) return (int64_t)m * ld;
  const uint32_t q = fdiv(m, f);
  return (int64_t)q * bs + (int64_t)(m - q * (uint32_t)mb) * ld;
}


__device__ __attribute__((aligned(32))) const unsigned g_zero_page[8] = {0u, 0u, 0u, 0u, 0u, 0u, 0u, 0u};

template <bool X3, bool CONV, bool F32>
struct StagerK {
  const void* base; int dtype; int K; int c;
  int64_t roff[4]; bool rok[4];
  uint64_t zpage;
  unsigned tapmask[4];
  int tap, ci, knext;
  Raw8<F32> raw[4];

  MTT_DEV void init(const GemmP& p, const void* b, int dt, int row0, int rows, int64_t ld, int mb, int64_t bs, FastDiv fmb) {
    base = b; dtype = dt; K = p.d.K; c = threadIdx.x & 7;
    zpage = (uint64_t)(uintptr_t)g_zero_page;
    asm volatile("" : "+s"(zpage));
#pragma unroll
    for (int i = 0; i < 4; ++i) {
      const int r = row0 + (threadIdx.x >> 3) + 32 * i;
      rok[i] = r < rows;
      const uint32_t rr = rok[i] ? (uint32_t)r : 0u;
      if (CONV) {
        const uint32_t t = fdiv(rr, p.divW);
        const int px = (int)(rr - t * (uint32_t)p.d.conv.W);
        const uint32_t bb = fdiv(t, p.divH);
        const int py = (int)(t - bb * (uint32_t)p.d.conv.H);
        roff[i] = (int64_t)rr * ld;
        unsigned m = 0;
#pragma unroll
        for (int tp = 0; tp < 9; ++tp) {
          int ty = tp / 3, tx = tp % 3;
          if (p.d.conv.flip) { ty = 2 - ty; tx = 2 - tx; }
          const int yy = py + (ty - 1) * p.d.conv.dil, xx = px + (tx - 1) * p.d.conv.dil;
          if (rok[i] && yy >= 0 && yy < p.d.conv.H && xx >= 0 && xx < p.d.conv.W) m |= 1u << tp;
        }
        tapmask[i] = m;
      } else {
        roff[i] = row_off(rr, mb, bs, ld, fmb);
        tapmask[i] = rok[i] ? 1u : 0u;
      }
    }
    ldx = ld;
    tap = 0; ci = c * 8; knext = 0;
    if (CONV) {
      while (ci >= p.d.conv.Cp) { ci -= p.d.conv.Cp; ++tap; }
    }
  }
  int64_t ldx;

  MTT_DEV void load(const GemmP& p, int k0) {
    const int k = k0 + c * 8;
    bool kok = k < K;
    int64_t koff = k;
    unsigned bit = 0;
    if (CONV) {
      if (k0 != knext) {
        const uint32_t t = fdiv((uint32_t)(kok ? k : 0), p.divCp);
        tap = (int)t; ci = k - (int)t * p.d.conv.Cp;
      }
      kok = kok && ci < p.d.conv.C;
      int ty = (int)fdiv((uint32_t)tap, p.div3), tx = tap - 3 * ty;
      if (p.d.conv.flip) { ty = 2 - ty; tx = 2 - tx; }
      koff = (int64_t)((ty - 1) * p.d.conv.dil * p.d.conv.W + (tx - 1) * p.d.conv.dil) * ldx + ci;
      bit = (unsigned)tap;
      ci += 64; knext = k0 + 64;
      while (ci >= p.d.conv.Cp) { ci -= p.d.conv.Cp; ++tap; }
    }
    const int es = F32 ? 4 : 2;
#pragma unroll
    for (int i = 0; i < 4; ++i) {
      const bool ok = kok && ((tapmask[i] >> bit) & 1u);
      const uint64_t real = (uint64_t)(uintptr_t)base + (uint64_t)((roff[i] + koff) * es);
      const unsigned char* ptr = (const unsigned char*)(uintptr_t)(ok ? real : zpage);
      if constexpr (F32) {
        raw[i].v0 = *(const float4*)ptr;
        raw[i].v1 = *(const float4*)(ptr + 16);
      } else {
        raw[i].r0 = *(const u32x4*)ptr;
      }
    }
  }
// ... 505 lines not shown
  __syncthreads();

  for (int kt = 0; kt < nk; ++kt) {
    const bool more = kt + 1 < nk;
    if (more) { sa.load(p, (kt + 1) * BK); sb.load(p, (kt + 1) * BK); }

    const unsigned char* st = smem + (kt & 1) * STAGE;
    const unsigned char* Ah = st;
    const unsigned char* Al = st + TILE_BYTES;
    const unsigned char* Bh = st + TILE_BYTES * NPL;
    const unsigned char* Bl = Bh + TILE_BYTES;
    if constexpr (!X3) {
      u32x4 fa[2][4], fb[2][4];
#pragma unroll
      for (int kh = 0; kh < 2; ++kh)
#pragma unroll
        for (int t = 0; t < 4; ++t) {
          fa[kh][t] = *(const u32x4*)(Ah + lds_off(wm * 64 + t * 16 + li, kh * 4 + lg));
          fb[kh][t] = *(const u32x4*)(Bh + lds_off(wn * 64 + t * 16 + li, kh * 4 + lg));
        }
      __builtin_amdgcn_sched_barrier(0);
#pragma unroll
      for (int kh = 0; kh < 2; ++kh)
#pragma unroll
        for (int a = 0; a < 4; ++a)
#pragma unroll
          for (int b = 0; b < 4; ++b) acc[a][b] = mfma16(fa[kh][a], fb[kh][b], acc[a][b]);
    } else {
#pragma unroll
      for (int kh = 0; kh < 2; ++kh) {
        u32x4 ah[4], al[4], bh[4], bl[4];
#pragma unroll
        for (int t = 0; t < 4; ++t) {
          const int ra = wm * 64 + t * 16 + li, rbn = wn * 64 + t * 16 + li;
          ah[t] = *(const u32x4*)(Ah + lds_off(ra, kh * 4 + lg));
          bh[t] = *(const u32x4*)(Bh + lds_off(rbn, kh * 4 + lg));
          al[t] = *(const u32x4*)(Al + lds_off(ra, kh * 4 + lg));
          bl[t] = *(const u32x4*)(Bl + lds_off(rbn, kh * 4 + lg));
        }
#pragma unroll
        for (int a = 0; a < 4; ++a)
#pragma unroll
          for (int b = 0; b < 4; ++b) {
            acc[a][b] = mfma16(al[a], bh[b], acc[a][b]);
            acc[a][b] = mfma16(ah[a], bl[b], acc[a][b]);
            acc[a][b] = mfma16(ah[a], bh[b], acc[a][b]);
          }
      }
    }

    if (more) {
      unsigned char* sn = smem + ((kt + 1) & 1) * STAGE;
      sa.store(sn, sn + TILE_BYTES);
      sb.store(sn + TILE_BYTES * NPL, sn + TILE_BYTES * NPL + TILE_BYTES);
    }
    __syncthreads();
  }

  gemm_epilogue_auto<BN, 2, 2, 4, 4, MODE != 3>(p, acc, smem, m0, n0, zo, zi);
}


MTT_DEV void glds16(const bf16_t* src, unsigned char* lds_wave_base) {
  __builtin_amdgcn_global_load_lds((const __attribute__((address_space(1))) void*)src,
                                   (__attribute__((address_space(3))) void*)lds_wave_base, 16, 0, 0);
}

constexpr int BM2 = 256;

template <int ADDR>
__global__ __launch_bounds__(512, 1) void gemm_dma_kernel(const GemmP p) {
  extern __shared__ __attribute__((aligned(16))) unsigned char smem[];
  constexpr int WAVES_N = 4, WAVES_M = 2, MT = 8, NT = 4;
  constexpr int TILE_A = BM2 * BK * 2, TILE_B = 256 * BK * 2, STAGE = TILE_A + TILE_B;
  constexpr bool FASTADDR = ADDR >= 1, X3CAT = ADDR == 2;
  MTT_TRACE_RT(0); MTT_TRACE(1);
  const int wg = xcd_remap(blockIdx.x, gridDim.x);
  const int tiles_n = (p.d.N + 255) / 256, tiles_m = (p.d.M + BM2 - 1) / BM2;
  int tile_m, tile_n;
  grouped_tile(wg, tiles_m, tiles_n, p.group_m, tile_m, tile_n);
  const int m0 = tile_m * BM2, n0 = tile_n * 256;
  const int z = blockIdx.z;
  const int zo = z / p.d.batch_inner, zi = z - zo * p.d.batch_inner;
  const int64_t za = (int64_t)zo * p.d.a_zo + (int64_t)zi * p.d.a_zi, zb = (int64_t)zo * p.d.b_zo + (int64_t)zi * p.d.b_zi;
  const bf16_t* Abase = (const bf16_t*)p.d.A + za;
  const bf16_t* Bbase = (const bf16_t*)p.d.B + zb;
  const bf16_t* AbaseL = X3CAT ? (const bf16_t*)p.d.A_lo + za : Abase;
  const bf16_t* BbaseL = X3CAT ? (const bf16_t*)p.d.B_lo + zb : Bbase;

  const int lane = threadIdx.x & 63, wave = __builtin_amdgcn_readfirstlane(threadIdx.x >> 6);
  const int li = lane & 15, lg = lane >> 4;
  const int wm = wave / WAVES_N, wn = wave % WAVES_N;
  const int late = wave >> 2;
  const int K = p.d.K;

  uint64_t zpage = (uint64_t)(uintptr_t)g_zero_page;
  asm volatile("" : "+s"(zpage));

  int64_t aoff[4], boff[4];
  int ack[4];
#pragma unroll
  for (int i = 0; i < 4; ++i) {
    const int row = (wave * 4 + i) * 8 + (lane >> 3);
    const int c = (lane & 7) ^ lds_swz(row);
    ack[i] = c * 8;
    int ra = m0 + row; if (ra > p.d.M - 1) ra = p.d.M - 1;
    aoff[i] = row_off((uint32_t)ra, p.d.a_mb, p.d.a_bs, p.d.lda, p.divAmb) + ack[i];
    int rb = n0 + row; if (rb > p.d.N - 1) rb = p.d.N - 1;
    boff[i] = (int64_t)rb * p.d.ldb + ack[i];
  }
  uint32_t aoff32[4], boff32[4];
  if constexpr (FASTADDR) {
#pragma unroll
    for (int i = 0; i < 4; ++i) { aoff32[i] = (uint32_t)aoff[i] * 2u; boff32[i] = (uint32_t)boff[i] * 2u; }
  }
  auto issue = [&](int stage, int s) {
    unsigned char* sA = smem + stage * STAGE + wave * 4096;
    unsigned char* sB = smem + stage * STAGE + TILE_A + wave * 4096;
    if constexpr (FASTADDR) {
      int t = s;
      const unsigned char* Ak = (const unsigned char*)Abase;
      const unsigned char* Bk = (const unsigned char*)Bbase;
      if constexpr (X3CAT) {
        t = (s * 21846) >> 16;
        const int j = s - 3 * t;
        if (j == 1) Ak = (const unsigned char*)AbaseL;
        if (j == 2) Bk = (const unsigned char*)BbaseL;
      }
      Ak += (size_t)t * (BK * 2);
      Bk += (size_t)t * (BK * 2);
#pragma unroll
      for (int i = 0; i < 4; ++i) glds16((const bf16_t*)(Ak + aoff32[i]), sA + i * 1024);
#pragma unroll
      for (int i = 0; i < 4; ++i) glds16((const bf16_t*)(Bk + boff32[i]), sB + i * 1024);
    } else {
      const int k0 = s * BK;
#pragma unroll
      for (int i = 0; i < 4; ++i) {
        const uint64_t src = (uint64_t)(uintptr_t)(Abase + (aoff[i] + k0));
        glds16((const bf16_t*)(uintptr_t)(k0 + ack[i] < K ? src : zpage), sA + i * 1024);
      }
#pragma unroll
      for (int i = 0; i < 4; ++i) {
        const uint64_t src = (uint64_t)(uintptr_t)(Bbase + (boff[i] + k0));
        glds16((const bf16_t*)(uintptr_t)(k0 + ack[i] < K ? src : zpage), sB + i * 1024);
      }
    }
  };

  f32x4 acc[MT][NT];
#pragma unroll
  for (int a = 0; a < MT; ++a)
#pragma unroll
    for (int b = 0; b < NT; ++b) acc[a][b] = (f32x4){0.f, 0.f, 0.f, 0.f};

  const int nk = X3CAT ? 3 * (K / BK) : (K + BK - 1) / BK;
  issue(0, 0);
  asm volatile("s_waitcnt vmcnt(0)" ::: "memory");
  __builtin_amdgcn_s_barrier();
  MTT_TRACE(2);
  if (late) __builtin_amdgcn_s_barrier();
  __builtin_amdgcn_sched_barrier(0);

  auto main_loop = [&](auto late_tag) {
  (void)late_tag;
  for (int kt = 0; kt < nk; ++kt) {
    const unsigned char* Ah = smem + (kt & 1) * STAGE;
    const unsigned char* Bh = Ah + TILE_A;
#pragma unroll
    for (int kh = 0; kh < 2; ++kh) {
      if (kh == 0 && kt + 1 < nk) issue((kt + 1) & 1, kt + 1);
      u32x4 fa[MT], fb[NT];
#pragma unroll
      for (int t = 0; t < NT; ++t) fb[t] = *(const u32x4*)(Bh + lds_off(wn * 64 + t * 16 + li, kh * 4 + lg));
#pragma unroll
      for (int t = 0; t < MT; ++t) fa[t] = *(const u32x4*)(Ah + lds_off(wm * (MT * 16) + t * 16 + li, kh * 4 + lg));
      if (kh == 1) asm volatile("s_waitcnt vmcnt(0) lgkmcnt(0)" ::: "memory");
      else asm volatile("s_waitcnt lgkmcnt(0)" ::: "memory");
      __builtin_amdgcn_sched_barrier(0);
      __builtin_amdgcn_s_barrier();
      __builtin_amdgcn_sched_barrier(0);
      __builtin_amdgcn_s_setprio(1);
#pragma unroll
      for (int a = 0; a < MT; ++a)
#pragma unroll
        for (int b = 0; b < NT; ++b) acc[a][b] = mfma16(fa[a], fb[b], acc[a][b]);
      __builtin_amdgcn_s_setprio(0);
      __builtin_amdgcn_sched_barrier(0);
      __builtin_amdgcn_s_barrier();
      __builtin_amdgcn_sched_barrier(0);
    }
  }
  };
  if (late) main_loop(std::true_type{}); else main_loop(std::false_type{});
  if (!late) __builtin_amdgcn_s_barrier();
  __syncthreads();
  MTT_TRACE(3);
  gemm_epilogue_auto<256, WAVES_M, WAVES_N, MT, NT>(p, acc, smem, m0, n0, zo, zi);
  MTT_TRACE(4); MTT_TRACE_RT(5); MTT_TRACE_ID(tile_m * tiles_n + tile_n);
}

template <int ADDR>
int launch_dma(const GemmP& p, hipStream_t stream) {
  constexpr int smem = (BM2 * BK * 2 + 256 * BK * 2) * 2;
  static std::atomic<unsigned long long> done{0};
  if (int e = mtt_ensure_dyn_lds((const void*)gemm_dma_kernel<ADDR>, smem, done)) return e;
  const int tm = (p.d.M + BM2 - 1) / BM2, tn = (p.d.N + 255) / 256;
  dim3 grid(tm * tn, 1, p.d.batch);
  hipLaunchKernelGGL((gemm_dma_kernel<ADDR>), grid, dim3(512), smem, stream, p);
  return (int)hipGetLastError();
}

MTT_DEV int ring_swz(int row) { return (0x78 >> (((row >> 2) & 3) * 2)) & 3; }

#define MTT_VMCNT_CASE(n) case n: asm volatile("s_waitcnt vmcnt(" #n ")" ::: "memory"); break;
MTT_DEV void wait_vmcnt_dyn(int n) {
  switch (n) {
    MTT_VMCNT_CASE(24) MTT_VMCNT_CASE(22) MTT_VMCNT_CASE(20) MTT_VMCNT_CASE(18) MTT_VMCNT_CASE(16) MTT_VMCNT_CASE(14) MTT_VMCNT_CASE(12)
    MTT_VMCNT_CASE(10) MTT_VMCNT_CASE(8) MTT_VMCNT_CASE(6) MTT_VMCNT_CASE(4) MTT_VMCNT_CASE(2)
    MTT_VMCNT_CASE(9) MTT_VMCNT_CASE(7) MTT_VMCNT_CASE(5) MTT_VMCNT_CASE(3) MTT_VMCNT_CASE(1)
    default: asm volatile("s_waitcnt vmcnt(0)" ::: "memory"); break;
  }
}

#ifndef MTT_R3_EDGE
#define MTT_R3_EDGE 1
#endif
template <int N_> MTT_DEV void wait_vmcnt_imm() { asm volatile("s_waitcnt vmcnt(%0)" :: "n"(N_) : "memory"); }

template <bool CONV, bool EDGE>
MTT_DEV void ring3_tile(const GemmP& p, unsigned char* smem, int m0, int n0, int zo, int zi) {
  constexpr int WAVES_N = EDGE ? 2 : 4, WAVES_M = EDGE ? 4 : 2, MT = EDGE ? 4 : 8, NT = 4;
  constexpr int NA = 2, NB = EDGE ? 1 : 2;
  constexpr int PART = 256 * 64, SLOT = 4 * PART;
  const int64_t za = (int64_t)zo * p.d.a_zo + (int64_t)zi * p.d.a_zi, zb = (int64_t)zo * p.d.b_zo + (int64_t)zi * p.d.b_zi;
  const unsigned char* AbaseH = (const unsigned char*)((const bf16_t*)p.d.A + za);
  const unsigned char* AbaseL = (const unsigned char*)((const bf16_t*)p.d.A_lo + za);
  const unsigned char* BbaseH = (const unsigned char*)((const bf16_t*)p.d.B + zb);
  const unsigned char* BbaseL = (const unsigned char*)((const bf16_t*)p.d.B_lo + zb);

  const int lane = threadIdx.x & 63, wave = __builtin_amdgcn_readfirstlane(threadIdx.x >> 6);
  const int li = lane & 15, lg = lane >> 4;
  const int wm = wave / WAVES_N, wn = wave % WAVES_N;
  const int late = wave >> 2;
  const int nk = p.d.K >> 5;

  uint32_t aoff32[2], boff32[2];
  unsigned tapmask[2] = {0x1ffu, 0x1ffu};
#pragma unroll
  for (int i = 0; i < 2; ++i) {
    const int row = (wave * 2 + i) * 16 + (lane >> 2);
    const int c = (lane & 3) ^ ring_swz(row);
    int ra = m0 + row; if (ra > p.d.M - 1) ra = p.d.M - 1;
    if constexpr (CONV) {
      aoff32[i] = (uint32_t)((int64_t)ra * p.d.lda + c * 8) * 2u;
      const uint32_t q = fdiv((uint32_t)ra, p.divW);
      const int px = ra - (int)q * p.d.conv.W;
      const int py = (int)q - (int)fdiv(q, p.divH) * p.d.conv.H;
      unsigned mk = 0;
#pragma unroll
      for (int t = 0; t < 9; ++t) {
        int ty = t / 3, tx = t - 3 * (t / 3);
        if (p.d.conv.flip) { ty = 2 - ty; tx = 2 - tx; }
        const int yy = py + (ty - 1) * p.d.conv.dil, xx = px + (tx - 1) * p.d.conv.dil;
        if (yy >= 0 && yy < p.d.conv.H && xx >= 0 && xx < p.d.conv.W) mk |= 1u << t;
      }
      tapmask[i] = mk;
    } else {
      aoff32[i] = (uint32_t)(row_off((uint32_t)ra, p.d.a_mb, p.d.a_bs, p.d.lda, p.divAmb) + c * 8) * 2u;
    }
    const int brow = EDGE ? wave * 16 + (lane >> 2) : row;
    const int cb = (lane & 3) ^ ring_swz(brow);
    int rb = n0 + brow; if (rb > p.d.N - 1) rb = p.d.N - 1;
    boff32[i] = (uint32_t)((int64_t)rb * p.d.ldb + cb * 8) * 2u;
  }
  uint64_t zpage = (uint64_t)(uintptr_t)g_zero_page;
  asm volatile("" : "+s"(zpage));
  const int cpt = CONV ? p.d.conv.Cp >> 5 : 1;
  const int cpt_inv = ((1 << 20) + cpt - 1) / cpt;
  auto issue_part = [&](int j, int part) {
    const bool isA = part == 0 || part == 3;
    unsigned char* dst = smem + (j & 1) * SLOT + part * PART + wave * ((EDGE && !isA) ? 1024 : 2048);
    if (CONV && isA) {
      const int tap = (j * cpt_inv) >> 20;
      int ty = (tap * 11) >> 5, tx = tap - 3 * ((tap * 11) >> 5);
      if (p.d.conv.flip) { ty = 2 - ty; tx = 2 - tx; }
      const int64_t delta = ((int64_t)((ty - 1) * p.d.conv.dil * p.d.conv.W + (tx - 1) * p.d.conv.dil) * p.d.lda + (int64_t)(j - tap * cpt) * 32) * 2;
      const unsigned char* base = (part == 0 ? AbaseH : AbaseL) + delta;
#pragma unroll
      for (int i = 0; i < 2; ++i) {
        const uint64_t src = (uint64_t)(uintptr_t)(base + aoff32[i]);
        glds16((const bf16_t*)(uintptr_t)(((tapmask[i] >> tap) & 1u) ? src : zpage), dst + i * 1024);
      }
      return;
    }
    const unsigned char* base = (part == 0 ? AbaseH : part == 1 ? BbaseH : part == 2 ? BbaseL : AbaseL) + (size_t)j * 64;
    glds16((const bf16_t*)(base + (isA ? aoff32[0] : boff32[0])), dst);
    if (isA || !EDGE) glds16((const bf16_t*)(base + (isA ? aoff32[1] : boff32[1])), dst + 1024);
  };
  const int fsw = ((lg ^ ring_swz(li)) << 4) + li * 64;
  const int fragA = wm * (MT * 16) * 64 + fsw, fragB = wn * (NT * 16) * 64 + fsw;

  f32x4 acc[MT][NT];
#pragma unroll
  for (int a = 0; a < MT; ++a)
#pragma unroll
    for (int b = 0; b < NT; ++b) acc[a][b] = (f32x4){0.f, 0.f, 0.f, 0.f};

  constexpr int W_BL = 3 * NA + 2 * NB, W_AL = 3 * NA + 3 * NB, W_AB = 2 * NA + 3 * NB;
  issue_part(0, 0); issue_part(0, 1); issue_part(0, 2); issue_part(0, 3);
  issue_part(1, 0); issue_part(1, 1); issue_part(1, 2);
  wait_vmcnt_imm<2 * NA + 3 * NB>();
  __builtin_amdgcn_s_barrier();
  if (late) __builtin_amdgcn_s_barrier();
  __builtin_amdgcn_sched_barrier(0);

#define MTT_R3_CLOSE() do { __builtin_amdgcn_sched_barrier(0); __builtin_amdgcn_s_barrier(); __builtin_amdgcn_sched_barrier(0); } while (0)
  auto main_loop = [&](auto late_tag) {
  constexpr bool LATE = decltype(late_tag)::value;
  for (int j = 0; j < nk; ++j) {
    const unsigned char* sb = smem + (j & 1) * SLOT;
    const bool m1 = j + 1 < nk, m2 = j + 2 < nk;
    const int w_bl = NA + (m1 ? 2 * NA + 2 * NB : 0), w_al = (m1 ? 2 * NA + 2 * NB : 0) + (m2 ? NA + NB : 0), w_ab = NA + NB + (m2 ? NA + 2 * NB : 0);
    u32x4 fa[MT], fbh[NT], fbl[NT];
    if (m1) issue_part(j + 1, 3);
#pragma unroll
    for (int t = 0; t < NT; ++t) fbh[t] = *(const u32x4*)(sb + PART + fragB + t * 1024);
#pragma unroll
    for (int t = 0; t < MT; ++t) fa[t] = *(const u32x4*)(sb + fragA + t * 1024);
    if (LATE) { if (m2) wait_vmcnt_imm<W_BL>(); else wait_vmcnt_dyn(w_bl); }
    asm volatile("s_waitcnt lgkmcnt(0)" ::: "memory");
    MTT_R3_CLOSE();
    __builtin_amdgcn_s_setprio(1);
#pragma unroll
    for (int a = 0; a < MT; ++a)
#pragma unroll
      for (int b = 0; b < NT; ++b) acc[a][b] = mfma16(fa[a], fbh[b], acc[a][b]);
    __builtin_amdgcn_s_setprio(0);
    if (!LATE) { if (m2) wait_vmcnt_imm<W_BL>(); else wait_vmcnt_dyn(w_bl); }
    MTT_R3_CLOSE();
    if (m2) { issue_part(j + 2, 0); issue_part(j + 2, 1); }
#pragma unroll
    for (int t = 0; t < NT; ++t) fbl[t] = *(const u32x4*)(sb + 2 * PART + fragB + t * 1024);
    if (LATE) { if (m2) wait_vmcnt_imm<W_AL>(); else wait_vmcnt_dyn(w_al); }
    asm volatile("s_waitcnt lgkmcnt(0)" ::: "memory");
    MTT_R3_CLOSE();
    __builtin_amdgcn_s_setprio(1);
#pragma unroll
    for (int a = 0; a < MT; ++a)
#pragma unroll
      for (int b = 0; b < NT; ++b) acc[a][b] = mfma16(fa[a], fbl[b], acc[a][b]);
    __builtin_amdgcn_s_setprio(0);
    if (!LATE) { if (m2) wait_vmcnt_imm<W_AL>(); else wait_vmcnt_dyn(w_al); }
    MTT_R3_CLOSE();
    if (m2) issue_part(j + 2, 2);
#pragma unroll
    for (int t = 0; t < MT; ++t) fa[t] = *(const u32x4*)(sb + 3 * PART + fragA + t * 1024);
    if (LATE) { if (m2) wait_vmcnt_imm<W_AB>(); else wait_vmcnt_dyn(w_ab); }
    asm volatile("s_waitcnt lgkmcnt(0)" ::: "memory");
    MTT_R3_CLOSE();
    __builtin_amdgcn_s_setprio(1);
#pragma unroll
    for (int a = 0; a < MT; ++a)
#pragma unroll
      for (int b = 0; b < NT; ++b) acc[a][b] = mfma16(fa[a], fbh[b], acc[a][b]);
    __builtin_amdgcn_s_setprio(0);
    if (!LATE) { if (m2) wait_vmcnt_imm<W_AB>(); else wait_vmcnt_dyn(w_ab); }
    MTT_R3_CLOSE();
  }
  };
#undef MTT_R3_CLOSE
  if (late) main_loop(std::true_type{}); else main_loop(std::false_type{});
  if (!late) __builtin_amdgcn_s_barrier();
  __syncthreads();
  if constexpr (EDGE) gemm_epilogue<128, WAVES_M, WAVES_N, MT, NT>(p, acc, smem, m0, n0, zo, zi);
  else gemm_epilogue_auto<256, WAVES_M, WAVES_N, MT, NT>(p, acc, smem, m0, n0, zo, zi);
}

template <bool CONV>
__global__ __launch_bounds__(512, 1) void gemm_ring3_kernel(const GemmP p) {
  extern __shared__ __attribute__((aligned(16))) unsigned char smem[];
  const int wg = xcd_remap(blockIdx.x, gridDim.x);
  const int tiles_n = (p.d.N + 255) / 256, tiles_m = (p.d.M + BM2 - 1) / BM2;
  int tile_m, tile_n;
  grouped_tile(wg, tiles_m, tiles_n, p.group_m, tile_m, tile_n);
  const int m0 = tile_m * BM2, n0 = tile_n * 256;
  const int z = blockIdx.z;
  const int zo = z / p.d.batch_inner, zi = z - zo * p.d.batch_inner;
  const int ncols = (p.d.n_store > p.d.N ? p.d.n_store : p.d.N) - n0;
  if (MTT_R3_EDGE && ncols <= 128 && p.d.store_mode == MTT_STORE_ROWS) ring3_tile<CONV, true>(p, smem, m0, n0, zo, zi);
  else ring3_tile<CONV, false>(p, smem, m0, n0, zo, zi);
}

template <bool CONV>
int launch_ring3(const GemmP& p, hipStream_t stream) {
  constexpr int smem = 2 * 4 * 16384;
  static std::atomic<unsigned long long> done{0};
  if (int e = mtt_ensure_dyn_lds((const void*)gemm_ring3_kernel<CONV>, smem, done)) return e;
  const int tm = (p.d.M + BM2 - 1) / BM2, tn = (p.d.N + 255) / 256;
  dim3 grid(tm * tn, 1, p.d.batch);
  hipLaunchKernelGGL((gemm_ring3_kernel<CONV>), grid, dim3(512), smem, stream, p);
  return (int)hipGetLastError();
}

template <bool EDGE>
MTT_DEV void ringc_tile(const GemmP& p, unsigned char* smem, int m0, int n0, int zo, int zi) {
  constexpr int WAVES_N = EDGE ? 2 : 4, WAVES_M = EDGE ? 4 : 2, MT = EDGE ? 4 : 8, NT = 4, S = 4;
  constexpr int NP = EDGE ? 3 : 4;
  constexpr int PART = 256 * 64, SLOT = 2 * PART;
  const unsigned char* Abase = (const unsigned char*)((const bf16_t*)p.d.A + ((int64_t)zo * p.d.a_zo + (int64_t)zi * p.d.a_zi));
  const unsigned char* Bbase = (const unsigned char*)((const bf16_t*)p.d.B + ((int64_t)zo * p.d.b_zo + (int64_t)zi * p.d.b_zi));

  const int lane = threadIdx.x & 63, wave = __builtin_amdgcn_readfirstlane(threadIdx.x >> 6);
  const int li = lane & 15, lg = lane >> 4;
  const int wm = wave / WAVES_N, wn = wave % WAVES_N;
  const int late = wave >> 2;
  const int nk = p.d.K >> 5;

  uint32_t aoff32[2], boff32[2];
  unsigned tapmask[2];
#pragma unroll
  for (int i = 0; i < 2; ++i) {
    const int row = (wave * 2 + i) * 16 + (lane >> 2);
    const int c = (lane & 3) ^ ring_swz(row);
    int ra = m0 + row; if (ra > p.d.M - 1) ra = p.d.M - 1;
    aoff32[i] = (uint32_t)((int64_t)ra * p.d.lda + c * 8) * 2u;
    const uint32_t q = fdiv((uint32_t)ra, p.divW);
    const int px = ra - (int)q * p.d.conv.W;
    const int py = (int)q - (int)fdiv(q, p.divH) * p.d.conv.H;
    unsigned mk = 0;
#pragma unroll
    for (int t = 0; t < 9; ++t) {
      int ty = t / 3, tx = t - 3 * (t / 3);
      if (p.d.conv.flip) { ty = 2 - ty; tx = 2 - tx; }
      const int yy = py + (ty - 1) * p.d.conv.dil, xx = px + (tx - 1) * p.d.conv.dil;
      if (yy >= 0 && yy < p.d.conv.H && xx >= 0 && xx < p.d.conv.W) mk |= 1u << t;
    }
    tapmask[i] = mk;
    const int brow = EDGE ? wave * 16 + (lane >> 2) : row;
    const int cb = (lane & 3) ^ ring_swz(brow);
    int rb = n0 + brow; if (rb > p.d.N - 1) rb = p.d.N - 1;
    boff32[i] = (uint32_t)((int64_t)rb * p.d.ldb + cb * 8) * 2u;
  }
  uint64_t zpage = (uint64_t)(uintptr_t)g_zero_page;
  asm volatile("" : "+s"(zpage));
  const int cpt = p.d.conv.Cp >> 5;
  const int cpt_inv = ((1 << 20) + cpt - 1) / cpt;
  auto issue_tile = [&](int j, int slot) {
    unsigned char* dst = smem + slot * SLOT + wave * 2048;
    const int tap = (j * cpt_inv) >> 20;
    int ty = (tap * 11) >> 5, tx = tap - 3 * ((tap * 11) >> 5);
    if (p.d.conv.flip) { ty = 2 - ty; tx = 2 - tx; }
    const int64_t delta = ((int64_t)((ty - 1) * p.d.conv.dil * p.d.conv.W + (tx - 1) * p.d.conv.dil) * p.d.lda + (int64_t)(j - tap * cpt) * 32) * 2;
    const unsigned char* abase = Abase + delta;
#pragma unroll
    for (int i = 0; i < 2; ++i) {
      const uint64_t src = (uint64_t)(uintptr_t)(abase + aoff32[i]);
      glds16((const bf16_t*)(uintptr_t)(((tapmask[i] >> tap) & 1u) ? src : zpage), dst + i * 1024);
    }
    const unsigned char* bbase = Bbase + (size_t)j * 64;
    if constexpr (EDGE) {
      glds16((const bf16_t*)(bbase + boff32[0]), smem + slot * SLOT + PART + wave * 1024);
    } else {
      glds16((const bf16_t*)(bbase + boff32[0]), dst + PART);
      glds16((const bf16_t*)(bbase + boff32[1]), dst + PART + 1024);
    }
  };
  const int fsw = ((lg ^ ring_swz(li)) << 4) + li * 64;
  const int fragA = wm * (MT * 16) * 64 + fsw, fragB = PART + wn * (NT * 16) * 64 + fsw;

  f32x4 acc[MT][NT];
#pragma unroll
  for (int a = 0; a < MT; ++a)
#pragma unroll
// ... 525 lines not shown
  return a_span < (1ll << 31) && b_span < (1ll << 31);
}
static int gemm_variant_for(const mtt_gemm_desc& d) {
  const bool any_split = d.a_dtype == MTT_SPLIT || d.b_dtype == MTT_SPLIT;
  if (any_split) {
    const bool both = d.prec == MTT_PREC_X3 && d.a_dtype == MTT_SPLIT && d.b_dtype == MTT_SPLIT && d.b_op == MTT_OP_K && d.A_lo && d.B_lo &&
                      d.store_mode == MTT_STORE_ROWS;
    if (d.a_scale) return MTT_E_UNSUPPORTED;
    if (both && d.a_op == MTT_OP_K && dma_fastaddr_ok(d, MTT_RING ? 32 : 64) && d.K >= 64 && d.K / 64 * 3 < 32768) return 8;
    if (both && d.a_op == MTT_OP_CONV_K && d.conv.Cp % 32 == 0 && d.conv.Cp <= 4096 && d.K == 9 * d.conv.Cp && d.a_mb <= 0 &&
        (int64_t)d.M * d.lda < (1ll << 31) && (int64_t)(d.N - 1) * d.ldb + d.K < (1ll << 31)) return 9;
    return MTT_E_UNSUPPORTED;
  }
  if (f32n_ok(d)) return 11;
  if (d.a_scale) return MTT_E_UNSUPPORTED;
  if (d.prec != MTT_PREC_BF16 || d.a_dtype != MTT_BF16 || d.b_dtype != MTT_BF16) return 0;
  if (d.a_op == MTT_OP_CONV_K && d.b_op == MTT_OP_K && d.variant != MTT_GEMM_GENERAL && d.store_mode == MTT_STORE_ROWS && d.conv.Cp % 32 == 0 &&
      d.conv.Cp <= 4096 && d.K == 9 * d.conv.Cp && d.lda == d.conv.Cp && d.a_mb <= 0 && (int64_t)d.M * d.lda < (1ll << 31) &&
      (int64_t)(d.N - 1) * d.ldb + d.K < (1ll << 31) && !d.colsum_out &&
      (d.variant == MTT_GEMM_DMA256 || (d.M >= 2048 && d.N >= 128))) return 12;
  const bool tn = d.a_op == MTT_OP_R && (d.b_op == MTT_OP_R || d.b_op == MTT_OP_CONV_R) && d.store_mode == MTT_STORE_ROWS;
  if (tn && d.variant != MTT_GEMM_GENERAL) {
    if (d.variant == MTT_GEMM_DMA256) return 6;
    const int64_t pm = (d.M + 255) / 256 * 256, pn = (d.N + 255) / 256 * 256;
    const int batch = d.batch < 1 ? 1 : d.batch;
    const bool fills = (pm / 256) * (pn / 256) * batch >= 64 && d.K >= 512;
    if (fills && 100 * (int64_t)d.M * d.N >= 45 * pm * pn) return 6;
    return 0;
  }
  const bool dma = d.a_op == MTT_OP_K && d.b_op == MTT_OP_K && (d.K % 8) == 0;
  if (!dma || d.variant == MTT_GEMM_GENERAL) return 0;
  if (d.variant == MTT_GEMM_DMA256) return 3;
  if (d.variant == MTT_GEMM_DMA128) return 4;
  const int n256 = (d.N + 255) / 256 * 256, n128 = (d.N + 127) / 128 * 128;
  const bool wide = 100 * n128 > 85 * n256;
  const int batch = d.batch < 1 ? 1 : d.batch;
  const int64_t blocks = (int64_t)((d.M + 255) / 256) * ((d.N + 255) / 256) * batch;
  if (wide && d.M >= 512 && d.N >= 512 && blocks >= 96) return 3;
  const int tbn = 32 * dma128_nt(d);
  const int64_t blocks128 = (int64_t)((d.M + 127) / 128) * ((d.N + tbn - 1) / tbn) * batch;
  if (d.M >= 512 && d.K >= 128 && blocks128 >= 256) return 4;
  if (d.M >= 128 && d.N >= 256 && d.K >= 512) return 4;
  return 0;
}
#ifdef MTT_GEMM_TRACE
static unsigned long long* g_trace_host = nullptr;
extern "C" void mtt_debug_set_trace(void* buf) { g_trace_host = (unsigned long long*)buf; }
#endif
extern "C" int mtt_gemm_variant(const mtt_gemm_desc* d) { return d ? gemm_variant_for(*d) : MTT_E_BADARG; }

static int gemm_launch(GemmP& p, hipStream_t s, int v);
extern "C" int mtt_gemm(const mtt_gemm_desc* dd, void* stream) {
  if (!dd || !dd->A || !dd->B || !dd->D) return MTT_E_BADARG;
  GemmP p; p.d = *dd;
  mtt_gemm_desc& d = p.d;
  if (d.M <= 0 || d.N <= 0 || d.K <= 0) return MTT_E_BADARG;
  if (d.batch < 1) d.batch = 1;
  if (d.batch_inner < 1) d.batch_inner = 1;
  const bool a_k = d.a_op == MTT_OP_K || d.a_op == MTT_OP_CONV_K, b_k = d.b_op == MTT_OP_K;
  const int Kp8 = (d.K + 7) / 8 * 8;
  if ((a_k && d.a_op == MTT_OP_K && d.lda < Kp8) || (b_k && d.ldb < Kp8)) return MTT_E_ALIGN;
  if (d.a_op == MTT_OP_CONV_K && (d.K % 8)) return MTT_E_ALIGN;
  if ((d.lda % 8) || (d.ldb % 8)) return MTT_E_ALIGN;
  if (((uintptr_t)d.A & 15) || ((uintptr_t)d.B & 15)) return MTT_E_ALIGN;
  if ((d.aux_in || d.aux_out) && (d.ldaux <= 0 || (d.ldaux % 8))) return MTT_E_BADARG;
  if (d.act < MTT_ACT_NONE || d.act > MTT_ACT_MUL_AUX) return MTT_E_BADARG;
  if ((d.act == MTT_ACT_GELU_DAUX && !d.aux_out) || ((d.act == MTT_ACT_MUL_AUX || d.act == MTT_ACT_GELU_BWD || d.act == MTT_ACT_RELU_BWD) && !d.aux_in))
    return MTT_E_BADARG;
  if ((d.ldd % 8) || ((uintptr_t)d.D & 15) || (d.d_bs % 8) || (d.d_zo % 8) || (d.d_zi % 8)) return MTT_E_ALIGN;
  if (d.resid && ((d.ldr % 4) || ((uintptr_t)d.resid & 15) || (d.r_bs % 4))) return MTT_E_ALIGN;
  const bool conv = d.a_op == MTT_OP_CONV_K || d.b_op == MTT_OP_CONV_R;
  if (conv) {
    if (d.conv.H <= 0 || d.conv.W <= 0 || d.conv.Cp % 8 || d.conv.C > d.conv.Cp || d.conv.dil < 1) return MTT_E_BADARG;
    if (d.a_op == MTT_OP_CONV_K && d.K != 9 * d.conv.Cp) return MTT_E_BADARG;
    if (d.b_op == MTT_OP_CONV_R && d.N != 9 * d.conv.Cp) return MTT_E_BADARG;
  }
  if (d.store_mode == MTT_STORE_PIXSHUF2 && (d.ps_H <= 0 || d.ps_W <= 0 || d.ps_Co <= 0 || d.N != 4 * d.ps_Co)) return MTT_E_BADARG;
  p.divW = make_div(conv ? d.conv.W : 1); p.divH = make_div(conv ? d.conv.H : 1);
  p.divCp = make_div(conv ? d.conv.Cp : 1); p.div3 = make_div(3);
  p.divAmb = make_div(d.a_mb > 0 ? d.a_mb : 1); p.divDmb = make_div(d.d_mb > 0 ? d.d_mb : 1);
  p.divRmb = make_div(d.r_mb > 0 ? d.r_mb : 1);
  p.divPsW = make_div(d.ps_W > 0 ? d.ps_W : 1); p.divPsH = make_div(d.ps_H > 0 ? d.ps_H : 1);
  p.divPsCo = make_div(d.ps_Co > 0 ? d.ps_Co : 1);
  p.tiles_m = (d.M + BM - 1) / BM; p.tiles_n = (d.N + BN - 1) / BN;
  p.group_m = MTT_GROUP_M;
#ifdef MTT_GEMM_TRACE
  p.trace = g_trace_host;
#endif
  hipStream_t s = (hipStream_t)stream;
  const int v = gemm_variant_for(d);
  if (v < 0) return v;
  if (d.d_dtype == MTT_SPLIT && !d.D_lo) return MTT_E_BADARG;
  if (d.d_dtype == MTT_SPLIT && d.store_mode != MTT_STORE_ROWS) return MTT_E_UNSUPPORTED;
  if (d.colsum_out) {
    if (!d.colsum_ws) return MTT_E_BADARG;
    if (d.batch != 1 || d.store_mode != MTT_STORE_ROWS || v == 6) return MTT_E_UNSUPPORTED;
    const int rc = gemm_launch(p, s, v);
    if (rc) return rc;
    const int tbm = (v == 3 || v == 8 || v == 9) ? 256 : BM;
    hipLaunchKernelGGL(mtt_colsum_final_kernel, dim3((d.N + 31) / 32, 1, 1), dim3(256), 0, s, (const float*)d.colsum_ws, d.colsum_out, d.N,
                       (d.M + tbm - 1) / tbm, (int64_t)0);
    return (int)hipGetLastError();
  }
  return gemm_launch(p, s, v);
}

extern "C" size_t mtt_gemm_colsum_ws_floats(const mtt_gemm_desc* d) {
  if (!d || d->M <= 0 || d->N <= 0) return 0;
  return (size_t)((d->M + BM - 1) / BM) * (size_t)((d->N + 7) / 8 * 8);
}

static int gemm_launch(GemmP& p, hipStream_t s, int v) {
  mtt_gemm_desc& d = p.d;
  if (v == 11) return launch_f32n(p, s);
  if (v == 12) return launch_ringc(p, s);
  if (v == 9) return launch_ring3<true>(p, s);
#if MTT_RING
  if (v == 8) return launch_ring3<false>(p, s);
#else
  if (v == 8) return launch_dma<2>(p, s);
#endif
  if (v == 3) return dma_fastaddr_ok(d) ? launch_dma<1>(p, s) : launch_dma<0>(p, s);
  if (v == 4) {
    const bool fa = dma_fastaddr_ok(d);
    switch (dma128_nt(d)) {
      case 1: return fa ? launch_dma128<true, 1>(p, s) : launch_dma128<false, 1>(p, s);
      case 2: return fa ? launch_dma128<true, 2>(p, s) : launch_dma128<false, 2>(p, s);
      default: return fa ? launch_dma128<true, 4>(p, s) : launch_dma128<false, 4>(p, s);
    }
  }
  if (v == 6) return d.b_op == MTT_OP_CONV_R ? launch_tn<true>(p, s) : launch_tn<false>(p, s);
  int mode;
  if (d.prec == MTT_PREC_X3) {
    if (d.a_dtype != MTT_F32 || d.b_dtype != MTT_F32) return MTT_E_UNSUPPORTED;
    mode = 2;
  } else if (d.a_dtype == MTT_BF16 && d.b_dtype == MTT_BF16) mode = 0;
  else if (d.a_dtype == MTT_F32 && d.b_dtype == MTT_BF16) mode = 1;
  else if (d.a_dtype == MTT_F32 && d.b_dtype == MTT_F32) { mode = 3; if (d.colsum_out) return MTT_E_UNSUPPORTED; }
  else if (d.a_dtype == MTT_BF16 && d.b_dtype == MTT_F32) mode = 4;
  else return MTT_E_UNSUPPORTED;
#define MTT_CASE(AO, BO) \
  if (d.a_op == AO && d.b_op == BO) \
    return mode == 2 ? launch<AO, BO, 2>(p, s) : (mode == 1 ? launch<AO, BO, 1>(p, s) : (mode == 3 ? launch<AO, BO, 3>(p, s) : (mode == 4 ? launch<AO, BO, 4>(p, s) : launch<AO, BO, 0>(p, s))));
  MTT_CASE(MTT_OP_K, MTT_OP_K)
  MTT_CASE(MTT_OP_K, MTT_OP_R)
  MTT_CASE(MTT_OP_R, MTT_OP_R)
  MTT_CASE(MTT_OP_CONV_K, MTT_OP_K)
  MTT_CASE(MTT_OP_R, MTT_OP_CONV_R)
#undef MTT_CASE
  return MTT_E_UNSUPPORTED;
}
```

multi-task-transformer_amd/ops.py:

```python
import weakref

import torch

from . import _lib
from ._lib import (ACT_GELU, ACT_NONE, ACT_RELU, BF16, F32, OP_CONV_K, OP_CONV_R, OP_K, OP_R, PREC_BF16, PREC_X3, SPLIT)


PITCH32_FROM = 160


def pitch(n):
    return (n + 31) // 32 * 32 if n >= PITCH32_FROM else (n + 7) // 8 * 8


DEFAULT_PREC = "x3f"


class Prec:

    def __init__(self, name):
        assert name in ("bf16", "x3", "x3f")
        self.name = name
        self.code = PREC_BF16 if name == "bf16" else PREC_X3
        self.adt = torch.bfloat16 if name == "bf16" else torch.float32
# ... 311 lines not shown
        return Split(torch.zeros(shape, dtype=torch.bfloat16, device=device), torch.zeros(shape, dtype=torch.bfloat16, device=device))
    return torch.zeros(shape, dtype=dtype, device=device)


def _mode(prec, split):
    return ('split', 'split') if split else (prec.name, prec.adt)


def pack_linear(weights, prec, tag, split=False):
    N, K = _w2d(weights[0])
    Kp, Z = pitch(K), len(weights)
    if not split and prec.adt == torch.float32 and Z == 1 and K == Kp and weights[0].is_contiguous():
        return weights[0].detach().reshape(1, N, K)
    mode, dt = _mode(prec, split)
    return seg_pack((tag, mode, tuple(id(w) for w in weights)), list(weights),
                    lambda: _dest((Z, N, Kp), dt, weights[0].device),
                    lambda buf: [segment(w, 0, buf, z * N * Kp, (1, N, K), (0, K, 1), (0, Kp, 1)) for z, w in enumerate(weights)],
                    check=lambda: _check_sources(weights, lambda w: _w2d(w) == (N, K)))


def pack_linear_T(weight, dtype, tag):
    N, K = _w2d(weight)
    return seg_pack((tag, 'wT', dtype, id(weight)), [weight], lambda: torch.zeros(K, N, dtype=dtype, device=weight.device),
                    lambda buf: [segment(weight, 0, buf, 0, (1, N, K), (0, K, 1), (0, 1, N))] if min(N, K) < 16 else
                                [segment(weight, 0, buf, 0, (1, K, N), (0, 1, K), (0, N, 1))],
                    check=lambda: _check_sources([weight], lambda w: True))


def pack_conv3(weights, prec, tag, transpose=False, split=None):
    Co, Ci = weights[0].shape[:2]
    if split is None:
        split = prec.split and split_conv_ok(Ci, Co)
    mode, dt = _mode(prec, split and not transpose)
    R, Cin = (Ci, Co) if transpose else (Co, Ci)
    Cp, Z = pitch(Cin), len(weights)
    s = (9, 1, Ci * 9) if transpose else (Ci * 9, 1, 9)
    return seg_pack((tag, mode, 'conv3', transpose, tuple(id(w) for w in weights)), list(weights),
                    lambda: _dest((Z, R, 9 * Cp), dt, weights[0].device),
                    lambda buf: [segment(w, 0, buf, z * R * 9 * Cp, (R, 9, Cin), s, (9 * Cp, Cp, 1)) for z, w in enumerate(weights)],
                    check=lambda: _check_sources(weights, lambda w: tuple(w.shape) == (Co, Ci, 3, 3)))


def split_conv_ok(Ci, Co=None):
    Cp = pitch(Ci)
    return Cp % 32 == 0 and Cp <= 4096 and (Co is None or Co * 9 * Cp < 2 ** 31)


def pack_upconv9(weights, prec, tag, split=False):
    Co, Ci = weights[0].shape[:2]
    Cop, Kp, Z = pitch(Co), pitch(Ci), len(weights)
    mode, dt = _mode(prec, split)
    return seg_pack((tag, mode, 'up9', tuple(id(w) for w in weights)), list(weights),
                    lambda: _dest((Z, 9 * Cop, Kp), dt, weights[0].device),
                    lambda buf: [segment(w, 0, buf, z * 9 * Cop * Kp, (9, Co, Ci), (1, Ci * 9, 9), (Cop * Kp, Kp, 1)) for z, w in enumerate(weights)],
                    check=lambda: _check_sources(weights, lambda w: tuple(w.shape) == (Co, Ci, 3, 3)))


def pack_kmap(weights, N, Kp, kmap, prec, tag, split=False):
    Z = len(weights)
    K = weights[0].numel() // N
    mode, dt = _mode(prec, split)
    return seg_pack((tag, mode, 'kmap', tuple(id(w) for w in weights)), list(weights),
                    lambda: _dest((Z, N, Kp), dt, weights[0].device),
                    lambda buf: [segment(w, s0, buf, z * N * Kp + d0, (1, N, ln), (0, K, 1), (0, Kp, 1))
                                 for z, w in enumerate(weights) for (d0, s0, ln) in kmap],
                    check=lambda: _check_sources(weights, lambda w: w.numel() == N * K))


def stack_vec(vs, tag):
    n, Z = vs[0].numel(), len(vs)
    if any(v.dtype != torch.float32 or not v.is_contiguous() or v.numel() != n for v in vs):
        def build():
            with torch.no_grad():
                return torch.stack([v.detach().float().reshape(-1) for v in vs], 0).contiguous()
        return _cached((tag, tuple(id(v) for v in vs)), vs, build)
    return seg_pack((tag, 'vec', tuple(id(v) for v in vs)), list(vs),
                    lambda: torch.zeros(Z, n, dtype=torch.float32, device=vs[0].device),
                    lambda buf: [segment(v, 0, buf, z * n, (1, 1, n), (0, 0, 1), (0, 0, 1)) for z, v in enumerate(vs)])



def linear(x, wpack, N, prec, *, bias=None, act=ACT_NONE, out=None, out_dtype=None, M=None,
           a_rows=None, d_rows=None, resid=None, r_rows=None, rowscale=None, n_prompt=0, aux_out=None, aux_in=None,
           colscale=None, alpha=1.0, batch_inner=1, d_z=None, ldd=None, n_store=None, a_affine=None):
    Z, Nw, Kp = wpack.shape
    assert N <= Nw
    x_split = isinstance(x, Split)
    assert x_split == isinstance(wpack, Split), "split planes: both operands or neither"
    if a_rows is not None:
        a_mb, a_bs, lda = a_rows
        a_z = 0
    else:
        xh = _hi(x)
        xv = xh if xh.dim() == 3 else xh[None]
        if M is None:
            M = xv.shape[1]
        a_mb, a_bs, lda = 0, 0, xv.shape[2]
        a_z = xv.stride(0) if xv.shape[0] > 1 else 0
        assert xv.shape[0] in (1, Z) and lda >= Kp
    Np = ldd if (out is None and ldd is not None) else pitch(N)
    if out is None:
        out = Split.empty((Z, M, Np), x.device) if out_dtype == "split" else torch.empty(Z, M, Np, dtype=out_dtype or prec.adt, device=x.device)
    oh = _hi(out)
    if d_rows is not None:
        d_mb, d_bs, ldd_ = d_rows
        dz = 0
        nst = N
    else:
        d_mb, d_bs = 0, 0
        ldd_ = ldd if ldd is not None else oh.shape[-1]
        dz = oh.stride(0) if oh.dim() == 3 else 0
        nst = min(Np, ldd_)
    if n_store is not None:
        nst = n_store
    wh = _hi(wpack)
    kw = dict(A=_hi(x), B=wh, D=oh, M=M, N=N, K=Kp, a_op=OP_K, b_op=OP_K,
              a_dtype=dtype_code(x), b_dtype=dtype_code(wpack), d_dtype=dtype_code(out), prec=prec.code,
              lda=lda, ldb=Kp, ldd=ldd_, a_mb=a_mb, a_bs=a_bs, d_mb=d_mb, d_bs=d_bs,
              batch=Z, batch_inner=batch_inner, alpha=alpha, act=act, n_store=nst)
    if x_split:
        kw.update(A_lo=x.lo, B_lo=wpack.lo)
    if isinstance(out, Split):
        kw.update(D_lo=out.lo)
    kw.update(a_zo=a_z * batch_inner, a_zi=a_z if batch_inner > 1 else 0,
              b_zo=wh.stride(0) * batch_inner, b_zi=wh.stride(0) if batch_inner > 1 else 0)
    if d_z is not None:
        kw.update(d_zo=d_z[0], d_zi=d_z[1])
    else:
        kw.update(d_zo=dz * batch_inner, d_zi=dz if batch_inner > 1 else 0)
    if bias is not None or colscale is not None:
        ref = bias if bias is not None else colscale
        cz = ref.stride(0) if (ref.dim() == 2 and ref.shape[0] > 1) else 0
        kw.update(colshift=bias, colscale=colscale, col_zo=cz * batch_inner, col_zi=cz if batch_inner > 1 else 0)
    if resid is not None:
        rr = r_rows if r_rows is not None else (d_mb, d_bs, ldd_)
        kw.update(resid=resid, r_mb=rr[0], r_bs=rr[1], ldr=rr[2])
    if rowscale is not None:
        kw.update(rowscale=rowscale, n_prompt=n_prompt)
    if aux_out is not None or aux_in is not None:
        aux = aux_out if aux_out is not None else aux_in
        az = aux.stride(0) if aux.dim() == 3 else 0
        kw.update(aux_out=aux_out, aux_in=aux_in, aux_dtype=dtype_code(aux), ldaux=aux.shape[-1],
                  aux_zo=az * batch_inner, aux_zi=az if batch_inner > 1 else 0)
    if a_affine is not None:
        sc, sh, a_act, a16 = a_affine
        kw.update(a_scale=sc, a_shift=sh, a_act=a_act, a_aux16=a16, ld_a16=a16.stride(-2) if a16 is not None else 0)
    call("gemm", **kw)
    return out


def head_prologue_ok(rows, K, n, lda):
    return GEMM_VARIANT is None and n <= 32 and K % 8 == 0 and K <= 1024 and rows >= 1 and lda % 4 == 0


SPLIT_CONV_MAX_ELEMS = 2 ** 31 - 1


def conv3x3(x, wpack, Co, Ci, B, H, W, prec, *, bias=None, colscale=None, act=ACT_NONE, dil=1, flip=0, out_dtype=None):
    Z, rows, Cp = x.shape
    assert rows == B * H * W and wpack.shape[-1] == 9 * Cp
    if isinstance(wpack, Split) and not isinstance(x, Split):
        x = x.float().contiguous()
        sp = split_cast(x.view(Z * rows, Cp))
        x = Split(sp.hi.view(Z, rows, Cp), sp.lo.view(Z, rows, Cp))
    assert isinstance(x, Split) == isinstance(wpack, Split), "split planes: both operands or neither"
    Cop = pitch(Co)
    if out_dtype == "split":
        assert isinstance(x, Split), "a split conv output needs the split-plane conv kernel"
        out = Split.empty((Z, rows, Cop), x.device)
    else:
        out = torch.empty(Z, rows, Cop, dtype=out_dtype or prec.adt, device=x.device)
    oh = _hi(out)
    per = max(1, SPLIT_CONV_MAX_ELEMS // (H * W * Cp)) if isinstance(x, Split) else B
    for b0 in range(0, B, per):
        nb = min(per, B - b0)
        r0, r1 = b0 * H * W, (b0 + nb) * H * W
        xa, xl = _hi(x)[:, r0:r1], (x.lo[:, r0:r1] if isinstance(x, Split) else None)
        kw = dict(A=xa, B=_hi(wpack), D=oh[:, r0:r1], M=r1 - r0, N=Co, K=9 * Cp, a_op=OP_CONV_K, b_op=OP_K,
                  a_dtype=dtype_code(x), b_dtype=dtype_code(wpack), d_dtype=dtype_code(out), prec=prec.code,
                  lda=Cp, ldb=9 * Cp, ldd=Cop, batch=Z, batch_inner=1, a_zo=_hi(x).stride(0), b_zo=_hi(wpack).stride(0), d_zo=oh.stride(0),
                  conv=dict(H=H, W=W, C=Ci, Cp=Cp, dil=dil, flip=flip), alpha=1.0, act=act, n_store=Cop)
        if isinstance(x, Split):
            kw.update(A_lo=xl, B_lo=wpack.lo)
        if isinstance(out, Split):
            kw.update(D_lo=out.lo[:, r0:r1])
        if bias is not None:
            kw.update(colshift=bias, col_zo=bias.stride(0))
        if colscale is not None:
            kw.update(colscale=colscale)
        call("gemm", **kw)
    return out


def upconv4_expand(z, C, B, h, w, *, bias=None, colscale=None, act=ACT_NONE):
    Z, rows, n9 = z.shape
    Cp = n9 // 9
    assert rows == B * h * w and n9 == 9 * Cp and z.is_contiguous()
    y = torch.empty(Z, B * 16 * h * w, Cp, dtype=z.dtype, device=z.device)
    call("upconv4_expand", z=z, y=y, bias=bias, colscale=colscale, Z=Z, B=B, h=h, w=w, C=C, Cp=Cp,
         z_dtype=dtype_code(z), y_dtype=dtype_code(y), act=act)
    return y


def upconv4_gather(dy, C, B, h, w):
    Z, rows, Cp = dy.shape
    assert rows == B * 16 * h * w and dy.is_contiguous()
    dz = torch.empty(Z, B * h * w, 9 * Cp, dtype=dy.dtype, device=dy.device)
    call("upconv4_gather", z=dz, y=dy, bias=None, colscale=None, Z=Z, B=B, h=h, w=w, C=C, Cp=Cp,
         z_dtype=dtype_code(dz), y_dtype=dtype_code(dy), act=ACT_NONE)
    return dz


def upconv3x3(x, w9, Co, B, h, w, prec, *, bias=None, colscale=None, act=ACT_NONE):
    if isinstance(w9, Split) and not isinstance(x, Split):
        Z, M, Kp = x.shape
        x = split_cast(x.reshape(Z * M, Kp))
        x = Split(x.hi.view(Z, M, Kp), x.lo.view(Z, M, Kp))
    z = linear(x, w9, w9.shape[1], prec, out_dtype=torch.float32 if isinstance(w9, Split) else None, ldd=w9.shape[1])
    return upconv4_expand(z, Co, B, h, w, bias=bias, colscale=colscale, act=act)


DECONV_SPLIT = True


def deconv2x2(x, wpack, Co, Ci, B, H, W, prec, *, bias4=None, out_dtype=None):
    Cop = pitch(Co)
    if (DECONV_SPLIT and prec.split and torch.is_tensor(x) and x.dtype == torch.float32 and x.dim() == 2 and x.is_contiguous()
            and wpack.dtype == torch.float32 and x.shape[1] == wpack.shape[-1] and split_gemm_ok(x.shape[1]) and B * H * W >= 2048):
        wsp = getattr(wpack, "_mtt_split", None)
        if wsp is None:
            wsp = wpack._mtt_split = split_cast(wpack[0].contiguous())
        z = linear(split_cast(x), Split(wsp.hi[None], wsp.lo[None]), 4 * Co, prec, bias=None if bias4 is None else bias4[None], out_dtype=torch.float32)
        out = torch.empty(B * 4 * H * W, Cop, dtype=out_dtype or prec.adt, device=x.device)
        call("pixshuf2", args=[z[0], out, B, H, W, Co, z.shape[-1], Cop, dtype_code(z), dtype_code(out)])
        return out
    out = torch.zeros(B * 4 * H * W, Cop, dtype=out_dtype or prec.adt, device=x.device)
    kw = dict(A=x, B=wpack, D=out, M=B * H * W, N=4 * Co, K=wpack.shape[-1], a_op=OP_K, b_op=OP_K,
              a_dtype=dtype_code(x), b_dtype=dtype_code(wpack), d_dtype=dtype_code(out), prec=prec.code,
              lda=x.shape[-1], ldb=wpack.shape[-1], ldd=Cop, batch=1, batch_inner=1, alpha=1.0, b_zo=0,
              store_mode=_lib.STORE_PIXSHUF2, ps_H=H, ps_W=W, ps_Co=Co)
    if bias4 is not None:
        kw.update(colshift=bias4)
    call("gemm", **kw)
    return out


def layernorm(x, gamma, beta, eps, prec, save_stats=False, out_dtype=None, want32=False):
    rows, C = x.shape
    split = out_dtype == "split"
    y = Split.empty((rows, C), x.device) if split else torch.empty(rows, C, dtype=out_dtype or prec.adt, device=x.device)
    mean = torch.empty(rows, dtype=torch.float32, device=x.device) if save_stats else None
    rstd = torch.empty(rows, dtype=torch.float32, device=x.device) if save_stats else None
    kw = {}
    y32 = None
    if split:
        kw.update(y_lo=y.lo)
        if want32:
            y32 = torch.empty(rows, C, dtype=torch.float32, device=x.device)
            kw.update(y32=y32, ldy32=C)
    call("layernorm_fwd", x=x, y=_hi(y), gamma=gamma, beta=beta, mean=mean, rstd=rstd, rows=rows, C=C,
         ldx=x.stride(0), ldy=C, y_dtype=dtype_code(y), eps=eps, **kw)
    return ((y, y32) if want32 else y), mean, rstd


def attention(qkv, B, N, nH, T, prec, want_lse=False):
    C = nH * 64
    split = isinstance(qkv, Split)
    out = Split.empty((B * N, C), qkv.device) if split else torch.empty(B * N, C, dtype=qkv.dtype, device=qkv.device)
    rawlog = torch.empty(B, nH, T, N, dtype=torch.float32, device=qkv.device) if T > 0 else None
    lse = torch.empty(B, nH, N, dtype=torch.float32, device=qkv.device) if want_lse else None
    kw = dict(qkv_lo=qkv.lo, out_lo=out.lo) if split else {}
    call("attn_fwd", qkv=_hi(qkv), out=_hi(out), rawlog=rawlog, lse=lse, B=B, N=N, nH=nH, T=T,
         dtype=dtype_code(qkv), prec=prec.code, scale=64 ** -0.5, **kw)
    return out, rawlog, lse


def patchify(img, prec):
    B, _, H, W = img.shape
    cols = torch.empty(B * (H // 16) * (W // 16), 768, dtype=prec.adt, device=img.device)
    call("patchify16", args=[img.contiguous(), cols, B, H, W, dtype_code(cols)])
    return cols


def chan_logits(cq, xn, B, T, N, C, grid, nwin_hw):
    nh, nw = nwin_hw
    rawchan = torch.empty(B, T, nh * nw, C, dtype=torch.float32, device=xn.device)
    kw = {}
    if isinstance(xn, Split):
        assert cq.dtype == torch.float32
        kw["xn_lo"] = xn.lo
    call("chan_logits", q=cq, xn=_hi(xn), rawchan=rawchan, B=B, T=T, N=N, C=C, h=grid[0], w=grid[1], nh=nh, nw=nw,
         dtype=dtype_code(xn), ldq=cq.shape[-1], ws=ws_for("chan_logits", xn.device, B=B, T=T, C=C, h=grid[0], w=grid[1], nh=nh, nw=nw), **kw)
    return rawchan


def prompt_rows32(xs, B, N, T, C):
    return (xs.hi.view(B, N, C)[:, :T].float() + xs.lo.view(B, N, C)[:, :T].float()).reshape(B * T, C)


def modulate(x, x_ld, x_bs, rawlog, rawchan, B, T, N, C, grid, nwin_hw, prec, hg=0, split=False):
    hw = grid[0] * grid[1]
    out = Split.empty((2 * T, B * hw, C), x.device) if split else torch.empty(2 * T, B * hw, C, dtype=prec.adt, device=x.device)
    call("modulate", x=x, x_ld=x_ld, x_bs=x_bs, rawlog=rawlog, rawchan=rawchan, out=_hi(out), out_lo=out.lo if split else None,
         B=B, T=T, N=N, C=C, h=grid[0], w=grid[1], nh=nwin_hw[0], nw=nwin_hw[1], out_dtype=dtype_code(out), hg=hg)
    return out


def split_gemm_ok(K):
    return K % 32 == 0 and K >= 64


def ctr_mix(fea, wmix, B, C, acc=None, out_dtype=torch.float32):
    T, rows, ld = fea.shape
    out = acc if acc is not None else torch.empty(T, rows, ld, dtype=out_dtype, device=fea.device)
    call("ctr_mix", fea=fea, out=out, wmix=wmix, T=T, B=B, rows_per_b=rows // B, ld=ld, C=ld,
         fea_dtype=dtype_code(fea), accumulate=1 if acc is not None else 0, out_dtype=dtype_code(out))
    return out


def ctr_weights(rawlog, w0, b0, w2, b2, B, T):
    nH, N = rawlog.shape[1], rawlog.shape[3]
    wmix = torch.empty(B, T, T, dtype=torch.float32, device=rawlog.device)
    call("ctr_weights", rawlog=rawlog, w0=w0, b0=b0, w2=w2, b2=b2, wmix=wmix, B=B, T=T, nH=nH, N=N)
    return wmix


def bilinear(x, B, C, Hin, Win, Hout, Wout, out_dtype, nchw=False):
    Z, _, ld = x.shape
    if nchw:
        out = torch.empty(B, C, Hout, Wout, dtype=torch.float32, device=x.device)
        call("bilinear_fwd", **{"in": x}, out=out, B=B, C=C, Hin=Hin, Win=Win, Hout=Hout, Wout=Wout, ld_in=ld, ld_out=0,
             in_dtype=dtype_code(x), out_dtype=F32, out_nchw=1, accumulate=0)
        return out
    out = torch.empty(Z, B * Hout * Wout, ld, dtype=out_dtype, device=x.device)
    call("bilinear_fwd", **{"in": x}, out=out, B=Z * B, C=ld, Hin=Hin, Win=Win, Hout=Hout, Wout=Wout, ld_in=ld, ld_out=ld,
         in_dtype=dtype_code(x), out_dtype=dtype_code(out), out_nchw=0, accumulate=0)
    return out


_ws_cache = {}
_ws_retired = []


def workspace(nfloats, device):
    key = (device.type, device.index)
    buf = _ws_cache.get(key)
    if buf is None or buf.numel() < nfloats:
        if device.type == "cuda" and torch.cuda.is_current_stream_capturing():
            raise RuntimeError("ops.workspace: the kernel workspace must not grow during stream capture; run one eager iteration of the same "
                               "shapes first (GraphedTrainStep's warm-up does)")
        if buf is not None:
            _ws_retired.append(buf)
        buf = torch.empty(max(int(nfloats), 1 << 18), dtype=torch.float32, device=device)
        _ws_cache[key] = buf
# ... 74 lines not shown
```

Baseline: 186.1.

## Skip GEMM and attention work for rows whose residual scale is zero

Adds a skip_scale descriptor to the GEMM and attention kernels. Tiles whose rows all carry a zero per-sample rowscale (patch or prompt part) skip the K loop or attention compute and write zeros. This covers the encoder block's forward and backward projection, MLP and flash attention paths, which avoids compute for samples whose branch contribution is dropped, such as under stochastic depth. The risk is that zeroed outputs change gradients if downstream consumers, like rawlog or channel paths, still need the true values. It also adds a per-tile check on the scale table.

Result: faster. 188.2, median of 6 (+1.1%).

```diff
diff --git a/include/mtt_hip.h b/include/mtt_hip.h
--- a/include/mtt_hip.h
+++ b/include/mtt_hip.h
@@ -66,6 +66,7 @@
   const void* A_lo; const void* B_lo; void* D_lo;
   float* colsum_out; float* colsum_ws;
   const float* a_scale; const float* a_shift; int32_t a_act; void* a_aux16; int64_t ld_a16;
+  const float* skip_scale; int32_t skip_mb; int32_t skip_prompt; int64_t skip_row0;
 } mtt_gemm_desc;
 size_t mtt_gemm_colsum_ws_floats(const mtt_gemm_desc* d);
 
@@ -81,6 +82,7 @@
   float scale;
   int32_t variant;
   const void* qkv_lo; void* out_lo;
+  const float* skip_scale;
 } mtt_attn_desc;
 int mtt_attn_fwd(const mtt_attn_desc* d, void* stream);
 int mtt_attn_bwd(const mtt_attn_desc* d, const void* dout, const float* drawlog, void* dqkv, float* stat, void* stream);
diff --git a/multi-task-transformer_amd/_lib.py b/multi-task-transformer_amd/_lib.py
--- a/multi-task-transformer_amd/_lib.py
+++ b/multi-task-transformer_amd/_lib.py
@@ -47,13 +47,14 @@
         ("A_lo", ptr), ("B_lo", ptr), ("D_lo", ptr),
         ("colsum_out", ptr), ("colsum_ws", ptr),
         ("a_scale", ptr), ("a_shift", ptr), ("a_act", i32), ("a_aux16", ptr), ("ld_a16", i64),
+        ("skip_scale", ptr), ("skip_mb", i32), ("skip_prompt", i32), ("skip_row0", i64),
     ]
 
 
 class AttnDesc(C.Structure):
     _fields_ = [("qkv", ptr), ("out", ptr), ("rawlog", ptr), ("lse", ptr),
                 ("B", i32), ("N", i32), ("nH", i32), ("T", i32), ("dtype", i32), ("prec", i32), ("scale", f32),
-                ("variant", i32), ("qkv_lo", ptr), ("out_lo", ptr)]
+                ("variant", i32), ("qkv_lo", ptr), ("out_lo", ptr), ("skip_scale", ptr)]
 
 
 class SoftmaxDesc(C.Structure):
diff --git a/multi-task-transformer_amd/autograd_path.py b/multi-task-transformer_amd/autograd_path.py
--- a/multi-task-transformer_amd/autograd_path.py
+++ b/multi-task-transformer_amd/autograd_path.py
@@ -165,6 +165,10 @@
     return _wgrad(dy, x, N, Kp, prec), db
 
 
+def _skip_kw(skip):
+    return {} if skip is None else dict(skip_scale=skip[0], skip_mb=skip[1], skip_prompt=skip[2])
+
+
 def _enc_dgrad(dy, weight, wpack2d, M, N_in, K_out, prec, out_dtype, tag, colsum=False, **epi):
     if colsum:
         if prec.name == "bf16" and (dy.dtype != torch.bfloat16 or wpack2d.dtype != torch.bfloat16):
@@ -240,13 +244,14 @@
 
 HEAD_DGRAD_DMA = True
 FLASH_BWD = True
-
-
-def attention_bwd_flash(qkv, ao, lse, dao, drawlog, B, N, nH, T, prec):
+DROP_SKIP = True
+
+
+def attention_bwd_flash(qkv, ao, lse, dao, drawlog, B, N, nH, T, prec, skip_scale=None):
     dqkv = torch.empty_like(qkv)
     dsum = torch.empty(B, nH, 2, (N + 3) // 4 * 4, dtype=torch.float32, device=qkv.device)
     ops.call("attn_bwd", qkv=qkv, out=ao, rawlog=None, lse=lse, B=B, N=N, nH=nH, T=T, dtype=dtype_code(qkv), prec=prec.code,
-             scale=64 ** -0.5, xargs=[dao, drawlog, dqkv, dsum])
+             scale=64 ** -0.5, xargs=[dao, drawlog, dqkv, dsum], **({} if skip_scale is None else dict(skip_scale=skip_scale)))
     return dqkv
 
 
@@ -268,6 +273,7 @@
     chan = Wtt is not None
     split = prec.split
     odt = "split" if split else prec.adt
+    skip = rowscale if DROP_SKIP else None
     xn, mean, rstd = ops.layernorm(XT, g1, b1, eps, prec, save_stats=keep, out_dtype=odt)
     wq = ops.pack_linear([Wqkv], pe, tag + ('qkv',), split=split)
     wp = ops.pack_linear([Wproj], pe, tag + ('proj',), split=split)
@@ -278,10 +284,10 @@
         ao16, rawlog, lse = ops.attention(q16, B, N, nH, T, pa)
         ao = ops.cast2d(ao16, ao16.shape[0], C, C, prec.adt, ldd=C)
     else:
-        ao, rawlog, lse = ops.attention(qkv, B, N, nH, T, pa, want_lse=flash)
+        ao, rawlog, lse = ops.attention(qkv, B, N, nH, T, pa, want_lse=flash, skip_scale=skip)
     XT2 = torch.empty_like(XT)
     rows = dict(d_rows=(N, N * C, C), M=B * N) if keep or rowscale is not None else {}
-    ops.linear(ao, wp, C, pe, bias=bproj[None], out=XT2, resid=XT, rowscale=rowscale, n_prompt=T, **rows)
+    ops.linear(ao, wp, C, pe, bias=bproj[None], out=XT2, resid=XT, rowscale=rowscale, n_prompt=T, skip=None if skip is None else (skip, N, T), **rows)
     cq = wt = wt1 = xp32 = rawchan = None
     if chan:
         wt = ops.pack_linear([Wtt], ps, tag + ('tt',))
@@ -312,10 +318,11 @@
     w2 = ops.pack_linear([W2], pe, tag + ('fc2',), split=split)
     z = torch.empty(B * N, Hd, dtype=prec.bwd.adt, device=XT2.device) if keep else None
     daux = keep and GELU_DAUX and z.dtype == torch.bfloat16
-    hmid = ops.linear(xn2, w1, Hd, pe, bias=b1[None], act=ACT_GELU_DAUX if daux else ACT_GELU, aux_out=z, out_dtype=odt)[0]
+    skip = (rowscale, N, T) if DROP_SKIP and rowscale is not None else None
+    hmid = ops.linear(xn2, w1, Hd, pe, bias=b1[None], act=ACT_GELU_DAUX if daux else ACT_GELU, aux_out=z, out_dtype=odt, skip=skip)[0]
     XT3 = torch.empty_like(XT2)
     rows = dict(d_rows=(N, N * C, C), M=B * N) if keep or rowscale is not None else {}
-    ops.linear(hmid, w2, C, pe, bias=b2[None], out=XT3, resid=XT2, rowscale=rowscale, n_prompt=T, **rows)
+    ops.linear(hmid, w2, C, pe, bias=b2[None], out=XT3, resid=XT2, rowscale=rowscale, n_prompt=T, skip=skip, **rows)
     saved = (XT2, g2, mean, rstd, ops._hi(xn2), z, ops._hi(hmid), ops._hi(w1), ops._hi(w2), rowscale) if keep else None
     return XT3, saved
 
@@ -343,11 +350,12 @@
             dXT2 = torch.zeros_like(XT)
         dXT2 = dXT2.contiguous()
         g, dbproj = _scaled_colsum(dXT2, rowscale, N, T, prec)
+        skip = (rowscale, N, T) if DROP_SKIP and rowscale is not None else None
         dWproj, _ = _enc_wgrad(g, ao, C, C, prec, bias=False)
-        dao = _enc_dgrad(g, Wproj_, wp[0], M, C, C, prec, prec.adt, 'proj')
+        dao = _enc_dgrad(g, Wproj_, wp[0], M, C, C, prec, prec.adt, 'proj', **_skip_kw(skip))
         dl = drawlog.contiguous() if (T > 0 and drawlog is not None and drawlog.numel()) else None
         if lse is not None:
-            dqkv = attention_bwd_flash(qkv, ao, lse, dao, dl, B, N, nH, T, prec)
+            dqkv = attention_bwd_flash(qkv, ao, lse, dao, dl, B, N, nH, T, prec, skip_scale=skip and skip[0])
         else:
             dqkv = attention_bwd(qkv, dao, dl, B, N, nH, T, prec)
         dWqkv, dbqkv = _enc_wgrad(dqkv, xn, 3 * C, C, prec)
@@ -407,11 +415,12 @@
         dXT3 = dXT3.contiguous()
         g, db2 = _scaled_colsum(dXT3, rowscale, N, T, prec)
         W1_, W2_ = ctx.params
+        skip = (rowscale, N, T) if DROP_SKIP and rowscale is not None else None
         dW2, _ = _enc_wgrad(g, hmid, C, Hd, prec, bias=False)
         dz, db1 = _enc_dgrad(g, W2_, w2[0], M, Hd, C, prec, prec.adt, 'fc2', colsum=True, act=ACT_MUL_AUX if ctx.daux else ACT_GELU_BWD, aux_in=z,
-                             aux_dtype=dtype_code(z), ldaux=Hd)
+                             aux_dtype=dtype_code(z), ldaux=Hd, **_skip_kw(skip))
         dW1, _ = _enc_wgrad(dz, xn2, Hd, C, prec, bias=False)
-        dxn2 = _enc_dgrad(dz, W1_, w1[0], M, C, Hd, prec, prec.adt, 'fc1')
+        dxn2 = _enc_dgrad(dz, W1_, w1[0], M, C, Hd, prec, prec.adt, 'fc1', **_skip_kw(skip))
         dXT2, dg2, dbn2 = _ln_bwd_join(dXT3, XT2, dxn2, g2, mean, rstd, ctx.eps)
         return dXT2, dg2, dbn2, None, dW1, db1, dW2, db2, None, None, None, None
 
diff --git a/multi-task-transformer_amd/csrc/attn_bwd.hip b/multi-task-transformer_amd/csrc/attn_bwd.hip
--- a/multi-task-transformer_amd/csrc/attn_bwd.hip
+++ b/multi-task-transformer_amd/csrc/attn_bwd.hip
@@ -21,7 +21,10 @@
   const bf16_t* qkv; const bf16_t* dout; const float* stat; const float* drawlog; bf16_t* dqkv;
   int B, N, nH, T, Np; float scale;
   const bf16_t* out; const float* lse; float* stat_w;
+  const float* skip_scale;
 };
+
+MTT_DEV bool bwd_patches_dead(const BwdP& p, int b) { return p.skip_scale != nullptr && p.skip_scale[2 * b + 1] == 0.0f; }
 
 MTT_DEV float dot8_bf16(const u32x4& a, const u32x4& g) {
   float s = 0.f;
@@ -120,6 +123,18 @@
   const int li = lane & 15, lg = lane >> 4;
   const int64_t tok0 = (int64_t)b * N;
   const int64_t bh = (int64_t)b * p.nH + h;
+  if (VER == 2 && qb * 128 >= p.T && bwd_patches_dead(p, b)) {
+#pragma unroll
+    for (int i = 0; i < 4; ++i) {
+      const int idx = tid + 256 * i, qrow = qb * 128 + (idx >> 3);
+      if (qrow < N) *(u32x4*)(p.dqkv + (tok0 + qrow) * 3 * C + h * HD + (idx & 7) * 8) = (u32x4){0u, 0u, 0u, 0u};
+    }
+    if (MTT_ABWD_DQSTAT && qb == nqb - 1 && tid < p.Np - N) {
+      p.stat_w[bh * 2 * p.Np + N + tid] = 0.f;
+      p.stat_w[bh * 2 * p.Np + p.Np + N + tid] = 0.f;
+    }
+    return;
+  }
   const int q0 = qb * 128 + wave * 32;
   const bool active = q0 < N;
 
@@ -545,8 +560,10 @@
   const float sc2 = p.scale * LOG2E, inv_scale = 1.0f / p.scale;
 
   const int nq = (N + 63) / 64;
+  int nlive = nq;
+  if (VER == 2 && bwd_patches_dead(p, b)) { const int np = (p.T + 63) / 64; nlive = np < nq ? np : nq; }
   if (VER == 2) {
-    dma_issue(smem, smem + STAT_LDS, 0);
+    if (nlive > 0) dma_issue(smem, smem + STAT_LDS, 0);
     asm volatile("s_waitcnt vmcnt(0)" ::: "memory");
   } else {
     stage_load(0);
@@ -557,7 +574,7 @@
   auto tile = [&](auto stage_tag, auto ragged_tag, auto first_tag, int j) {
     constexpr int ST = decltype(stage_tag)::value;
     constexpr int RG = decltype(ragged_tag)::value, FT = decltype(first_tag)::value;
-    const bool more = RG != 1 && j + 1 < nq;
+    const bool more = RG != 1 && j + 1 < nlive;
     if (more) {
       if (VER == 2) dma_issue(smem + (1 - ST) * STAGE, smem + STAT_LDS + (1 - ST) * STAT_STAGE, (j + 1) * 64);
       else stage_load((j + 1) * 64);
@@ -716,13 +733,16 @@
   };
   if (VER == 2 && MTT_ABWD_TILES) {
     const int nfull = N / 64;
-    if (nfull >= 1) tile(BwdNo{}, BwdNo{}, BwdYes{}, 0);
-    else tile(BwdNo{}, BwdYes{}, BwdYes{}, 0);
-    for (int j = 1; j < nfull; j += 2) {
+    const int nlf = nfull < nlive ? nfull : nlive;
+    if (nlive >= 1) {
+      if (nfull >= 1) tile(BwdNo{}, BwdNo{}, BwdYes{}, 0);
+      else tile(BwdNo{}, BwdYes{}, BwdYes{}, 0);
+    }
+    for (int j = 1; j < nlf; j += 2) {
       tile(BwdYes{}, BwdNo{}, BwdNo{}, j);
-      if (j + 1 < nfull) tile(BwdNo{}, BwdNo{}, BwdNo{}, j + 1);
-    }
-    if (nfull >= 1 && nfull < nq) {
+      if (j + 1 < nlf) tile(BwdNo{}, BwdNo{}, BwdNo{}, j + 1);
+    }
+    if (nfull >= 1 && nfull < nq && nlive == nq) {
       if (nfull & 1) tile(BwdYes{}, BwdYes{}, BwdNo{}, nfull);
       else tile(BwdNo{}, BwdYes{}, BwdNo{}, nfull);
     }
@@ -775,7 +795,7 @@
     hipLaunchKernelGGL(attn_stat_kernel, dim3((unsigned)((chunks + 255) / 256)), dim3(256), 0, s, (const bf16_t*)d->out, (const bf16_t*)dout,
                        d->lse, stat, d->B, d->N, d->nH, Np);
   BwdP p{(const bf16_t*)d->qkv, (const bf16_t*)dout, stat, d->T > 0 ? drawlog : nullptr, (bf16_t*)dqkv, d->B, d->N, d->nH, d->T, Np, d->scale,
-         (const bf16_t*)d->out, d->lse, stat};
+         (const bf16_t*)d->out, d->lse, stat, d->skip_scale};
   dim3 grid((unsigned)(((d->N + 127) / 128) * d->nH * d->B));
   if (ver == 0) {
     hipLaunchKernelGGL(attn_bwd_dq_kernel<0>, grid, dim3(256), smem_dq, s, p);
diff --git a/multi-task-transformer_amd/csrc/attn_fast.hip b/multi-task-transformer_amd/csrc/attn_fast.hip
--- a/multi-task-transformer_amd/csrc/attn_fast.hip
+++ b/multi-task-transformer_amd/csrc/attn_fast.hip
@@ -19,6 +19,22 @@
 MTT_DEV void attn_glds16(const bf16_t* src, unsigned char* lds_wave_base) {
   __builtin_amdgcn_global_load_lds((const __attribute__((address_space(1))) void*)src,
                                    (__attribute__((address_space(3))) void*)lds_wave_base, 16, 0, 0);
+}
+MTT_DEV bool attn_block_dead(const mtt_attn_desc& d, int b, int qb) {
+  return d.skip_scale != nullptr && qb * 128 >= d.T && d.skip_scale[2 * b + 1] == 0.0f;
+}
+MTT_DEV void attn_store_dead_block(const mtt_attn_desc& d, int b, int h, int qb) {
+  const int N = d.N, C = d.nH * HD, tid = threadIdx.x;
+  const u32x4 z = (u32x4){0u, 0u, 0u, 0u};
+#pragma unroll
+  for (int i = 0; i < 4; ++i) {
+    const int idx = tid + 256 * i, qrow = qb * 128 + (idx >> 3);
+    if (qrow >= N) continue;
+    const int64_t oi = ((int64_t)b * N + qrow) * C + h * HD + (idx & 7) * 8;
+    *(u32x4*)((bf16_t*)d.out + oi) = z;
+    if (d.out_lo) *(u32x4*)((bf16_t*)d.out_lo + oi) = z;
+  }
+  if (d.lse && tid < 128 && qb * 128 + tid < N) d.lse[((int64_t)b * d.nH + h) * N + qb * 128 + tid] = 0.f;
 }
 template <int OFF>
 MTT_DEV u32x2 attn_ds_read_tr16(unsigned addr) {
@@ -35,6 +51,7 @@
   const int wi = xcd_remap(blockIdx.x, gridDim.x);
   const int qb = wi % nqb, bh = wi / nqb;
   const int h = bh % d.nH, b = bh / d.nH;
+  if (VER == 2 && attn_block_dead(d, b, qb)) { attn_store_dead_block(d, b, h, qb); return; }
   const int N = d.N, C = d.nH * HD;
   const int tid = threadIdx.x, lane = tid & 63, wave = tid >> 6;
   const int li = lane & 15, lg = lane >> 4;
@@ -369,6 +386,7 @@
   const int wi = xcd_remap(blockIdx.x, gridDim.x);
   const int qb = wi % nqb, bh = wi / nqb;
   const int h = bh % d.nH, b = bh / d.nH;
+  if (attn_block_dead(d, b, qb)) { attn_store_dead_block(d, b, h, qb); return; }
   const int N = d.N, C = d.nH * HD;
   const int tid = threadIdx.x, lane = tid & 63, wave = tid >> 6;
   const int li = lane & 15, lg = lane >> 4;
diff --git a/multi-task-transformer_amd/csrc/gemm.hip b/multi-task-transformer_amd/csrc/gemm.hip
--- a/multi-task-transformer_amd/csrc/gemm.hip
+++ b/multi-task-transformer_amd/csrc/gemm.hip
@@ -17,6 +17,7 @@
   FastDiv divW, divH, divCp, div3;
   FastDiv divAmb, divDmb, divRmb;
   FastDiv divPsW, divPsH, divPsCo;
+  FastDiv divSkip;
   int tiles_m, tiles_n;
   int group_m;
 #ifdef MTT_GEMM_TRACE
@@ -44,6 +45,19 @@
   if (mb <= 0) return (int64_t)m * ld;
   const uint32_t q = fdiv(m, f);
   return (int64_t)q * bs + (int64_t)(m - q * (uint32_t)mb) * ld;
+}
+
+MTT_DEV bool skip_rows_dead(const GemmP& p, uint32_t r0, uint32_t r1) {
+  const uint32_t mb = (uint32_t)p.d.skip_mb, np = (uint32_t)p.d.skip_prompt;
+  uint32_t q = fdiv(r0, p.divSkip);
+  uint32_t o = r0 - q * mb;
+  for (uint32_t r = r0; r < r1;) {
+    const uint32_t c = o >= np ? 1u : 0u;
+    if (p.d.skip_scale[2 * q + c] != 0.0f) return false;
+    if (c) { r += mb - o; ++q; o = 0; }
+    else { r += np - o; o = np; if (np == mb) { ++q; o = 0; } }
+  }
+  return true;
 }
 
 
@@ -715,6 +729,8 @@
   const int m0 = tile_m * BM2, n0 = tile_n * 256;
   const int z = blockIdx.z;
   const int zo = z / p.d.batch_inner, zi = z - zo * p.d.batch_inner;
+  const bool dead = ADDR == 1 && p.d.skip_scale != nullptr &&
+                    skip_rows_dead(p, (uint32_t)m0, (uint32_t)(m0 + BM2 < p.d.M ? m0 + BM2 : p.d.M));
   const int64_t za = (int64_t)zo * p.d.a_zo + (int64_t)zi * p.d.a_zi, zb = (int64_t)zo * p.d.b_zo + (int64_t)zi * p.d.b_zi;
   const bf16_t* Abase = (const bf16_t*)p.d.A + za;
   const bf16_t* Bbase = (const bf16_t*)p.d.B + zb;
@@ -787,8 +803,8 @@
 #pragma unroll
     for (int b = 0; b < NT; ++b) acc[a][b] = (f32x4){0.f, 0.f, 0.f, 0.f};
 
-  const int nk = X3CAT ? 3 * (K / BK) : (K + BK - 1) / BK;
-  issue(0, 0);
+  const int nk = dead ? 0 : X3CAT ? 3 * (K / BK) : (K + BK - 1) / BK;
+  if (!dead) issue(0, 0);
   asm volatile("s_waitcnt vmcnt(0)" ::: "memory");
   __builtin_amdgcn_s_barrier();
   MTT_TRACE(2);
@@ -862,7 +878,7 @@
 template <int N_> MTT_DEV void wait_vmcnt_imm() { asm volatile("s_waitcnt vmcnt(%0)" :: "n"(N_) : "memory"); }
 
 template <bool CONV, bool EDGE>
-MTT_DEV void ring3_tile(const GemmP& p, unsigned char* smem, int m0, int n0, int zo, int zi) {
+MTT_DEV void ring3_tile(const GemmP& p, unsigned char* smem, int m0, int n0, int zo, int zi, bool dead) {
   constexpr int WAVES_N = EDGE ? 2 : 4, WAVES_M = EDGE ? 4 : 2, MT = EDGE ? 4 : 8, NT = 4;
   constexpr int NA = 2, NB = EDGE ? 1 : 2;
   constexpr int PART = 256 * 64, SLOT = 4 * PART;
@@ -876,7 +892,7 @@
   const int li = lane & 15, lg = lane >> 4;
   const int wm = wave / WAVES_N, wn = wave % WAVES_N;
   const int late = wave >> 2;
-  const int nk = p.d.K >> 5;
+  const int nk = dead ? 0 : p.d.K >> 5;
 
   uint32_t aoff32[2], boff32[2];
   unsigned tapmask[2] = {0x1ffu, 0x1ffu};
@@ -941,8 +957,10 @@
     for (int b = 0; b < NT; ++b) acc[a][b] = (f32x4){0.f, 0.f, 0.f, 0.f};
 
   constexpr int W_BL = 3 * NA + 2 * NB, W_AL = 3 * NA + 3 * NB, W_AB = 2 * NA + 3 * NB;
-  issue_part(0, 0); issue_part(0, 1); issue_part(0, 2); issue_part(0, 3);
-  issue_part(1, 0); issue_part(1, 1); issue_part(1, 2);
+  if (!dead) {
+    issue_part(0, 0); issue_part(0, 1); issue_part(0, 2); issue_part(0, 3);
+    issue_part(1, 0); issue_part(1, 1); issue_part(1, 2);
+  }
   wait_vmcnt_imm<2 * NA + 3 * NB>();
   __builtin_amdgcn_s_barrier();
   if (late) __builtin_amdgcn_s_barrier();
@@ -1021,8 +1039,10 @@
   const int z = blockIdx.z;
   const int zo = z / p.d.batch_inner, zi = z - zo * p.d.batch_inner;
   const int ncols = (p.d.n_store > p.d.N ? p.d.n_store : p.d.N) - n0;
-  if (MTT_R3_EDGE && ncols <= 128 && p.d.store_mode == MTT_STORE_ROWS) ring3_tile<CONV, true>(p, smem, m0, n0, zo, zi);
-  else ring3_tile<CONV, false>(p, smem, m0, n0, zo, zi);
+  const bool dead = !CONV && p.d.skip_scale != nullptr &&
+                    skip_rows_dead(p, (uint32_t)m0, (uint32_t)(m0 + BM2 < p.d.M ? m0 + BM2 : p.d.M));
+  if (MTT_R3_EDGE && ncols <= 128 && p.d.store_mode == MTT_STORE_ROWS) ring3_tile<CONV, true>(p, smem, m0, n0, zo, zi, dead);
+  else ring3_tile<CONV, false>(p, smem, m0, n0, zo, zi, dead);
 }
 
 template <bool CONV>
@@ -1714,6 +1734,10 @@
   p.divRmb = make_div(d.r_mb > 0 ? d.r_mb : 1);
   p.divPsW = make_div(d.ps_W > 0 ? d.ps_W : 1); p.divPsH = make_div(d.ps_H > 0 ? d.ps_H : 1);
   p.divPsCo = make_div(d.ps_Co > 0 ? d.ps_Co : 1);
+  if (d.skip_scale) {
+    if (d.skip_mb <= 0 || d.skip_prompt < 0 || d.skip_prompt > d.skip_mb || d.skip_row0 < 0) return MTT_E_BADARG;
+  }
+  p.divSkip = make_div(d.skip_scale ? d.skip_mb : 1);
   p.tiles_m = (d.M + BM - 1) / BM; p.tiles_n = (d.N + BN - 1) / BN;
   p.group_m = MTT_GROUP_M;
 #ifdef MTT_GEMM_TRACE
diff --git a/multi-task-transformer_amd/ops.py b/multi-task-transformer_amd/ops.py
--- a/multi-task-transformer_amd/ops.py
+++ b/multi-task-transformer_amd/ops.py
@@ -417,7 +417,7 @@
 
 def linear(x, wpack, N, prec, *, bias=None, act=ACT_NONE, out=None, out_dtype=None, M=None,
            a_rows=None, d_rows=None, resid=None, r_rows=None, rowscale=None, n_prompt=0, aux_out=None, aux_in=None,
-           colscale=None, alpha=1.0, batch_inner=1, d_z=None, ldd=None, n_store=None, a_affine=None):
+           colscale=None, alpha=1.0, batch_inner=1, d_z=None, ldd=None, n_store=None, a_affine=None, skip=None):
     Z, Nw, Kp = wpack.shape
     assert N <= Nw
     x_split = isinstance(x, Split)
@@ -477,6 +477,8 @@
         az = aux.stride(0) if aux.dim() == 3 else 0
         kw.update(aux_out=aux_out, aux_in=aux_in, aux_dtype=dtype_code(aux), ldaux=aux.shape[-1],
                   aux_zo=az * batch_inner, aux_zi=az if batch_inner > 1 else 0)
+    if skip is not None:
+        kw.update(skip_scale=skip[0], skip_mb=skip[1], skip_prompt=skip[2])
     if a_affine is not None:
         sc, sh, a_act, a16 = a_affine
         kw.update(a_scale=sc, a_shift=sh, a_act=a_act, a_aux16=a16, ld_a16=a16.stride(-2) if a16 is not None else 0)
@@ -598,13 +600,15 @@
     return ((y, y32) if want32 else y), mean, rstd
 
 
-def attention(qkv, B, N, nH, T, prec, want_lse=False):
+def attention(qkv, B, N, nH, T, prec, want_lse=False, skip_scale=None):
     C = nH * 64
     split = isinstance(qkv, Split)
     out = Split.empty((B * N, C), qkv.device) if split else torch.empty(B * N, C, dtype=qkv.dtype, device=qkv.device)
     rawlog = torch.empty(B, nH, T, N, dtype=torch.float32, device=qkv.device) if T > 0 else None
     lse = torch.empty(B, nH, N, dtype=torch.float32, device=qkv.device) if want_lse else None
     kw = dict(qkv_lo=qkv.lo, out_lo=out.lo) if split else {}
+    if skip_scale is not None:
+        kw.update(skip_scale=skip_scale)
     call("attn_fwd", qkv=_hi(qkv), out=_hi(out), rawlog=rawlog, lse=lse, B=B, N=N, nH=nH, T=T,
          dtype=dtype_code(qkv), prec=prec.code, scale=64 ** -0.5, **kw)
     return out, rawlog, lse
```
